# UBCMOCCA/mocca_envs

Hardware: AMD Instinct MI355X
Metric: env-steps/sec, Walker3DCustomEnv-v0 @ 4096 envs, 1/2/4/8 MI355X (higher is better)
Workload: dtype f32; 1 GPU; Walker3DCustomEnv-v0, 4096 envs/GPU, flat ground, U(-1,1) action tape, auto-reset; max_rows=48, max_contacts=12, envs_per_gpu=4096, parallelism=independent env shards x1, no collective, preroll_steps=6344

## Files before the change

### include/mocca.h

```cpp
#ifndef MOCCA_H
#define MOCCA_H

#include <stddef.h>
#include <stdint.h>

#include "mocca_model.h"

#ifdef __cplusplus
extern "C" {
#endif

#define MOCCA_ABI_VERSION 8

typedef struct mocca_ctx *mocca_handle;

enum {
  MOCCA_OK = 0,
  MOCCA_E_ARG = -1,
  MOCCA_E_HIP = -2,
  MOCCA_E_TOPOLOGY = -3,
  MOCCA_E_NODEVICE = -4,
};

enum {
  MOCCA_PARAM_AUTO_RESET = 0,
  MOCCA_PARAM_EVAL_MODE = 1,
  MOCCA_PARAM_CURRICULUM = 2,
  MOCCA_PARAM_RANDOM_POSE = 3,
  MOCCA_PARAM_HOST_RETARGET = 4,
  MOCCA_PARAM_SEED = 5,
  MOCCA_PARAM_ENV_OFFSET = 6,
  MOCCA_PARAM_RANDOM_REWARD = 8,
  MOCCA_PARAM_APPLIED_GAIN = 7,
  MOCCA_PARAM_ISSUE_PRIORITY = 9,
  MOCCA_PARAM_PERSIST_IMPULSES = 10,
  MOCCA_PARAM_KERNEL_VARIANT = 11,
  MOCCA_PARAM_ORDER_EVERY = 12,
  MOCCA_PARAM_PACE_TICKS = 13,
};

#define MOCCA_DEBUG_WORDS 20
enum {
  MOCCA_DBG_ROWS = 0,
  MOCCA_DBG_LIMIT_ROWS = 1,
  MOCCA_DBG_CONTACTS = 2,
  MOCCA_DBG_SLOTS_LO = 3,
  MOCCA_DBG_SLOTS_HI = 4,
  MOCCA_DBG_LIMITS_LO = 5,
  MOCCA_DBG_LIMITS_HI = 6,
  MOCCA_DBG_SELF = 7,
  MOCCA_DBG_CLAMP_LO = 8,
  MOCCA_DBG_CLAMP_HI = 9,
  MOCCA_DBG_CLAMPSIG_LO = 10,
  MOCCA_DBG_CLAMPSIG_HI = 11,
  MOCCA_DBG_CAP_CONTACTS = 12,
  MOCCA_DBG_CAP_ROWS = 13,
  MOCCA_DBG_SUBSTEPS = 14,
  MOCCA_DBG_ROWS_WANTED = 15,
  MOCCA_DBG_STEPSIG_LO = 16,
  MOCCA_DBG_STEPSIG_HI = 17,
  MOCCA_DBG_STEPSIG_N = 18,
  MOCCA_DBG_RESERVED = 19,
};

int mocca_abi_version(void);
size_t mocca_model_sizeof(void);

int mocca_create(const void *model_blob, size_t nbytes, int task_id, int n_envs, int device, mocca_handle *out);
int mocca_destroy(mocca_handle h);

int mocca_n_envs(mocca_handle h);
int mocca_obs_dim(mocca_handle h);
int mocca_act_dim(mocca_handle h);
int mocca_plan_dim(mocca_handle h);
int mocca_state_dim(mocca_handle h);

int mocca_reset(mocca_handle h, const uint8_t *mask_dev, uint64_t seed, float *obs_dev, void *stream);

int mocca_step(mocca_handle h, const float *act_dev, float *obs_dev, float *rew_dev, uint8_t *done_dev,
               int32_t *info_dev, void *stream);

int mocca_task_step(mocca_handle h, const float *act_dev, const int32_t *touch_dev, const int32_t *target_dev,
                    const int32_t *body_dev, float *obs_dev, float *rew_dev, uint8_t *done_dev, int32_t *info_dev,
                    void *stream);

int mocca_set_draw_tape(mocca_handle h, const float *tape_dev, int n_per_env);

int mocca_observe(mocca_handle h, float *obs_dev, void *stream);

int mocca_get_state(mocca_handle h, float *state_dev, void *stream);
int mocca_set_state(mocca_handle h, const float *state_dev, void *stream);
int mocca_get_task(mocca_handle h, uint32_t *task_dev, void *stream);
int mocca_set_task(mocca_handle h, const uint32_t *task_dev, void *stream);
int mocca_get_terrain(mocca_handle h, float *terrain_dev, void *stream);
int mocca_set_terrain(mocca_handle h, const float *terrain_dev, void *stream);

int mocca_set_param(mocca_handle h, int param_id, double value);
int mocca_set_param_v(mocca_handle h, int param_id, const float *values_dev, int broadcast, void *stream);
int mocca_set_seed(mocca_handle h, uint64_t seed);
int mocca_set_debug_buffer(mocca_handle h, int32_t *dbg_dev);
int mocca_set_terminal_obs_buffer(mocca_handle h, float *final_obs_dev);
typedef struct mocca_episode_rec {
  uint32_t serial;
  float ret;
  int32_t length;
  uint32_t flags;
} mocca_episode_rec;
int mocca_set_episode_stats(mocca_handle h, float *masks_dev, float *bad_masks_dev, float *totals_dev, void *records, int n_slots,
                            size_t slot_stride_bytes);
uint32_t mocca_episode_serial(mocca_handle h);

int mocca_is_diagnostic_build(void);

int mocca_set_trajectory(mocca_handle h, const float *table_host, int n_frames, double max_time, double control_step);

int mocca_set_heightfield(mocca_handle h, const float *heights_host, int rows, int cols, double scale);

#define MOCCA_HF_MAX_FIELDS 1024
#define MOCCA_HF_MAX_PEAKS 256
int mocca_set_heightfield_bank(mocca_handle h, const float *heights_host, int n_fields, int rows, int cols, double scale);
int mocca_generate_heightfields(mocca_handle h, int first, int count, uint64_t seed, int n_peaks, double gain, void *stream);
// ... 146 lines not shown
```

### mocca_envs_amd/csrc/mocca_api.hip

```cpp
#include <hip/hip_runtime.h>

#include <cmath>
#include <cstdio>
#include <cstring>
#include <functional>
#include <memory>
#include <new>
#include <string>
#include <utility>
#include <vector>

#include "mocca.h"
#include "mocca_kernels.h"
#include "mocca_optim.h"
#include "mocca_policy.h"
#include "mocca_ppo.h"
#include "mocca_render.h"
#include "mocca_rollout.h"
#include "mocca_scan.h"
#include "mocca_depth.h"
#include "mocca_terrain.h"
#include "mocca_randomise.h"

using namespace mocca;

extern "C" size_t mocca_r32_args_sizeof(void);
extern "C" int mocca_r32_max_rows(void);
extern "C" int mocca_r32_max_contacts(void);
extern "C" void mocca_r32_launch_step(int topo, int task_id, int n, hipStream_t s, const void* args);
extern "C" void mocca_r32_kernel_info(int topo, int task_id, hipFuncAttributes* fa, int* nb, hipError_t* e);
extern "C" size_t mocca_r64_args_sizeof(void);
extern "C" int mocca_r64_max_rows(void);
extern "C" int mocca_r64_max_contacts(void);
extern "C" void mocca_r64_launch_step(int topo, int task_id, int n, hipStream_t s, const void* args);
extern "C" void mocca_r64_kernel_info(int topo, int task_id, hipFuncAttributes* fa, int* nb, hipError_t* e);

__global__ void copy_param_kernel(float* dst, const float* src, bool broadcast, int n) {
  const int i = blockIdx.x * blockDim.x + threadIdx.x;
  if (i < n) dst[i] = src[broadcast ? 0 : i];
}
__global__ void set_task_word_kernel(uint32_t* task, int word, const float* vals, float scalar, int use_scalar, int n) {
  const int i = blockIdx.x * blockDim.x + threadIdx.x;
  if (i < n) task[(size_t)i * MOCCA_TASK_WORDS + word] = __float_as_uint(use_scalar ? scalar : vals[i]);
}

__global__ __launch_bounds__(1024) void order_by_rows_kernel(const uint32_t* task, int32_t* order, int n) {
  __shared__ int hist[64], start[64];
  const int t = threadIdx.x;
  if (t < 64) hist[t] = 0;
  __syncthreads();
  for (int e = t; e < n; e += 1024) {
    const uint32_t r = task[(size_t)e * MOCCA_TASK_WORDS + MOCCA_TW_LAST_ROWS];
    atomicAdd(&hist[63 - (r > 63u ? 63u : r)], 1);
  }
  __syncthreads();
  if (t == 0) {
    int acc = 0;
    for (int k = 0; k < 64; ++k) { start[k] = acc; acc += hist[k]; }
  }
  __syncthreads();
  for (int e = t; e < n; e += 1024) {
    const uint32_t r = task[(size_t)e * MOCCA_TASK_WORDS + MOCCA_TW_LAST_ROWS];
    order[atomicAdd(&start[63 - (r > 63u ? 63u : r)], 1)] = e;
  }
}

template <class T>
class DevBuf {
  T* p_ = nullptr;

 public:
  DevBuf() = default;
  DevBuf(DevBuf&& o) noexcept : p_(std::exchange(o.p_, nullptr)) {}
  DevBuf& operator=(DevBuf&& o) noexcept { swap(o); return *this; }
  ~DevBuf() { reset(); }
  void reset() {
    if (p_) (void)hipFree(p_);
    p_ = nullptr;
  }
  void swap(DevBuf& o) noexcept { std::swap(p_, o.p_); }
  hipError_t alloc(size_t count, bool zero) {
    reset();
    hipError_t e = hipMalloc(&p_, count * sizeof(T));
    if (e != hipSuccess) { p_ = nullptr; return e; }
    if (zero && (e = hipMemset(p_, 0, count * sizeof(T))) != hipSuccess) reset();
    return e;
  }
  T* get() const { return p_; }
  operator T*() const { return p_; }
};

struct mocca_ctx {
  MoccaModel model;
  int task_id = 0, n_envs = 0, device = 0, obs_dim = 0;
  DevBuf<MoccaModel> d_model;
  int topo = 0;
  DevBuf<float> d_dyn;
  DevBuf<uint32_t> d_task;
  DevBuf<float> d_terrain;
  int auto_reset = 0, eval_mode = 0, random_pose = 1, curriculum = 0, host_retarget = 0, env_offset = 0, random_reward = 0;
  float gain = 1.0f;
  bool compact = false;
  bool wide = false;
  int force_full = 0;
  bool delassus_valu = false;
  int persist_warm = 0;
  int pace = -18;
  DevBuf<unsigned long long> d_pace_acc;
  DevBuf<float> d_ep_ret;
  float *ep_masks = nullptr, *ep_bad = nullptr, *ep_totals = nullptr;
  char* ep_rec = nullptr;
  int ep_slots = 0;
  size_t ep_stride = 0;
  uint32_t ep_serial = 1;
  int order_every = 0;
  int order_age = 0;
  DevBuf<int32_t> d_order;
  bool gain_pending = false;
  float* final_obs = nullptr;
  DevBuf<float> d_pvec[3];
  bool pvec_on[3] = {false, false, false};
  const float* tape = nullptr;
  int tape_n = 0;
  int32_t* dbg = nullptr;
  int prio = MOCCA_PRIO_T1 + 64 * MOCCA_PRIO_T2 + 4096 * MOCCA_PRIO_T3;
  uint64_t seed = 0;
  DevBuf<float> d_traj;
  int traj_n = 0;
  double traj_tmax = 0.0, traj_cstep = 0.0;
  DevBuf<float> d_hf;
  int hf_rows = 0, hf_cols = 0, hf_n_fields = 0, hf_planes = 1;
  float hf_scale = 0.0f;
  DevBuf<float> d_hf_range;
  DevBuf<float> d_hf_part;
  DevBuf<int32_t> d_hf_field;
  int hf_redraw = 0;
  DevBuf<float> d_scenes;
  int scenes_cap = 0;
  DevBuf<float> d_scan_pts;
  int scan_n = 0;
  float scan_above = 0.0f, scan_drop = 0.0f;
  bool depth_on = false;
  mocca_depth::DepthArgs depth{};
  DevBuf<float> d_ctrl_image;
  DevBuf<int32_t> d_ctrl_layers;
  mocca_ctrl::ControllerArgs ctrl{};
  DevBuf<float> d_robot_state;
  DevBuf<float> d_base_act;
  DevBuf<float> d_base_val;
  DevBuf<float> d_ctrl_norm;
  struct PolicySlot {
    DevBuf<float> d_pol_image;
    DevBuf<int32_t> d_pol_layers;
    mocca_pol::PolicyArgs pol{};
    mocca_pol::RepackArgs pol_repack{};
    size_t pol_n_base = 0;
    bool pol_filled = false;
    int pol_tail_row = 0;
    std::vector<int32_t> pol_table;
    int pol_wt_off[mocca_ppo::PPO_MAX_TABLE] = {};
  } student, teacher;
  struct {
    mocca_ppo::PpoMode method = mocca_ppo::PPO_PLAIN;
    DevBuf<int32_t> perm;
    DevBuf<float> sign;
    double coef = 0.0;
  } pol_mirror;
  const float* critic_rows = nullptr;
  int critic_stride = 0;
  DevBuf<double> d_gae_part;
  size_t gae_part_cap = 0;
  DevBuf<double> d_obs_part;
  size_t obs_part_cap = 0;
  DevBuf<double> d_ppo;
  size_t ppo_cap = 0;
  DevBuf<double> d_optim;
  size_t optim_cap = 0;
  bool rand_on = false;
  mocca_rand::RandConfig rand_cfg{};
  DevBuf<float> d_rand_eff;
  DevBuf<float> d_rand_ring;
  DevBuf<float> d_noise_scale;
  std::string err;
};
static_assert(ROBOT_STATE_STRIDE == mocca_ctrl::CTRL_RS_STRIDE, "the step kernels and the controller kernel share the robot_state buffer");

static thread_local std::string g_err;

// ... 245 lines not shown
  int rc = check_topology(h->model, task_id, &h->topo, g_err);
  if (rc != MOCCA_OK) return rc;
  int ndev = 0;
  if (hipGetDeviceCount(&ndev) != hipSuccess || ndev <= 0 || device < 0 || device >= ndev) { g_err = "no such HIP device"; return MOCCA_E_NODEVICE; }
  h->task_id = task_id; h->n_envs = n_envs; h->device = device;
  h->compact = compact_ok(h->model, h->topo);
  h->wide = wide_needed(h->model);
  if (h->wide && mocca_r64_args_sizeof() != sizeof(StepArgs)) { g_err = "the 64-row kernel instance was built from another StepArgs"; return MOCCA_E_ARG; }
  if (h->compact) h->pace = 0;
  h->obs_dim = task_id == MOCCA_TASK_CASSIE
                   ? (h->model.cassie_mode == MOCCA_CASSIE_PLAIN ? 6 + 2 * h->model.n_ordered + 2 : 12 + 2 * h->model.n_ordered + 2)
                   : 6 + 2 * h->model.n_joints + h->model.n_feet + (task_id == MOCCA_TASK_WALKER3D_STEPPER ? 5 * (h->model.lookbehind + 2) : 2);
  if (task_id == MOCCA_TASK_CASSIE && (h->model.cassie_mode < MOCCA_CASSIE_PLAIN || h->model.cassie_mode > MOCCA_CASSIE_PHASE_MIRROR ||
                                       (h->model.cassie_mode != MOCCA_CASSIE_PLAIN && h->model.n_ordered != 14))) {
    g_err = "Cassie blob: unknown cassie_mode (the mocap / phase envs need the 14 ordered joints)"; return MOCCA_E_ARG;
  }
  if (task_id == MOCCA_TASK_WALKER3D_STEPPER &&
      (h->model.n_planks < 1 || h->model.n_planks > MOCCA_MAX_PLANKS || h->model.lookbehind < 1 || h->model.lookbehind > 2)) {
    g_err = "Stepper blob: n_planks must be 1..4 and lookbehind 1 or 2"; return MOCCA_E_ARG;
  }
  auto fail = [&](const char* what, hipError_t e) {
    g_err = std::string(what) + ": " + hipGetErrorString(e);
    return MOCCA_E_HIP;
  };
  hipError_t e;
  DeviceGuard guard(device);
  if ((e = guard.err) != hipSuccess) return fail("hipSetDevice", e);
  if ((e = h->d_model.alloc(1, false)) != hipSuccess) return fail("hipMalloc(model)", e);
  if ((e = hipMemcpy(h->d_model, &h->model, sizeof(MoccaModel), hipMemcpyHostToDevice)) != hipSuccess) return fail("hipMemcpy(model)", e);
  const size_t n = (size_t)n_envs;
  if ((e = h->d_dyn.alloc(n * DYN_STRIDE, false)) != hipSuccess) return fail("hipMalloc(state)", e);
  if ((e = h->d_task.alloc(n * MOCCA_TASK_WORDS, false)) != hipSuccess) return fail("hipMalloc(task)", e);
  if ((e = h->d_terrain.alloc(n * TERRAIN_STRIDE, true)) != hipSuccess) return fail("hipMalloc(terrain)", e);
  if ((e = h->d_pace_acc.alloc(1, true)) != hipSuccess) return fail("hipMalloc(pace samples)", e);
  {
    std::vector<uint32_t> tmp(n * MOCCA_TASK_WORDS);
    const float one = 1.0f;
    uint32_t one_bits; std::memcpy(&one_bits, &one, 4);
    for (size_t i = 0; i < n; ++i) {
      tmp[i * MOCCA_TASK_WORDS + MOCCA_TW_EPISODE] = (uint32_t)-1;
      tmp[i * MOCCA_TASK_WORDS + MOCCA_TW_APPLIED_GAIN] = one_bits;
    }
    if ((e = hipMemcpy(h->d_task, tmp.data(), tmp.size() * sizeof(uint32_t), hipMemcpyHostToDevice)) != hipSuccess) return fail("hipMemcpy(task)", e);
  }
  {
    std::vector<float> tmp(n * DYN_STRIDE);
    for (size_t i = 0; i < n; ++i) tmp[i * DYN_STRIDE + 6] = 1.0f;
    if ((e = hipMemcpy(h->d_dyn, tmp.data(), tmp.size() * sizeof(float), hipMemcpyHostToDevice)) != hipSuccess) return fail("hipMemcpy(state)", e);
  }
  *out = h.release();
  return MOCCA_OK;
} catch (const std::bad_alloc&) { return out_of_host_memory(nullptr, "mocca_create"); }

int mocca_destroy(mocca_handle h) {
  delete h;
  return MOCCA_OK;
}

int mocca_n_envs(mocca_handle h) { return h ? h->n_envs : MOCCA_E_ARG; }
int mocca_obs_dim(mocca_handle h) { return h ? h->obs_dim : MOCCA_E_ARG; }
int mocca_act_dim(mocca_handle h) {
  if (!h) return MOCCA_E_ARG;
  return h->task_id == MOCCA_TASK_CASSIE ? h->model.n_ctrl - 2 : h->model.n_joints;
}
int mocca_plan_dim(mocca_handle h) {
  if (!h) return MOCCA_E_ARG;
  if (h->task_id != MOCCA_TASK_WALKER3D_PLANNER) { h->err = "mocca_plan_dim: only the planner task takes plans"; return MOCCA_E_ARG; }
  return mocca_ctrl::CTRL_PLAN;
}
int mocca_state_dim(mocca_handle h) { return h ? MOCCA_STATE_DIM(h->model.n_joints, h->model.n_slots) : MOCCA_E_ARG; }

static StepArgs make_args(mocca_handle h) {
  StepArgs a{};
  a.model = h->d_model; a.dyn = h->d_dyn; a.task = h->d_task; a.terrain = h->d_terrain;
  a.n_envs = h->n_envs; a.obs_dim = h->obs_dim;
  a.auto_reset = h->auto_reset; a.eval_mode = h->eval_mode; a.random_pose = h->random_pose; a.curriculum = h->curriculum;
  a.host_retarget = h->host_retarget; a.env_offset = h->env_offset; a.random_reward = h->random_reward;
  a.seed_lo = (uint32_t)h->seed; a.seed_hi = (uint32_t)(h->seed >> 32);
  a.curriculum_v = h->pvec_on[0] ? h->d_pvec[0].get() : nullptr;
  a.eval_mode_v = h->pvec_on[1] ? h->d_pvec[1].get() : nullptr;
  a.gain_v = h->pvec_on[2] ? h->d_pvec[2].get() : nullptr;
  a.gain = h->gain;
  a.dbg = h->dbg;
  a.prio = h->prio | (h->delassus_valu ? PRIO_DELASSUS_VALU : 0);
  a.traj = h->d_traj; a.traj_n = h->traj_n; a.traj_tmax = h->traj_tmax; a.traj_cstep = h->traj_cstep;
  a.final_obs = h->final_obs;
  a.persist_warm = h->persist_warm;
  a.pace = h->pace;
  a.pace_acc = h->d_pace_acc;
  a.ep_ret = h->d_ep_ret; a.ep_masks = h->ep_masks; a.ep_bad = h->ep_bad; a.ep_totals = h->ep_totals;
  a.hf = h->d_hf; a.hf_rows = h->hf_rows; a.hf_cols = h->hf_cols; a.hf_scale = h->hf_scale;
  if (h->hf_n_fields > 1) {
    a.hf_field = h->d_hf_field; a.hf_stride = h->hf_planes * h->hf_rows * h->hf_cols; a.hf_n_fields = h->hf_n_fields; a.hf_redraw = h->hf_redraw;
  }
  a.robot_state = h->d_ctrl_image ? h->d_robot_state.get() : nullptr;
  return a;
}
static int flush_pending(mocca_handle h, hipStream_t s) {
  if (!h->gain_pending) return MOCCA_OK;
  launch_per_env(set_task_word_kernel, h, s, h->d_task, MOCCA_TW_APPLIED_GAIN, nullptr, h->gain, 1, h->n_envs);
  HIP_TRY(h, hipGetLastError());
  h->gain_pending = false;
  return MOCCA_OK;
}
static int need_heightfield(mocca_handle h, const char* who, const char* when) {
  if (h->task_id != MOCCA_TASK_WALKER3D_PLANNER || h->d_hf) return MOCCA_OK;
  h->err = std::string(who) + "the planner task needs mocca_set_heightfield " + when;
  return MOCCA_E_ARG;
}
static mocca_rdr::HeightFieldBank heightfield_record(mocca_handle h) {
  if (h->task_id != MOCCA_TASK_WALKER3D_PLANNER) return mocca_rdr::HeightFieldBank{nullptr, 0, 0, 0.0f, nullptr, nullptr, 0};
  return mocca_rdr::HeightFieldBank{h->d_hf, h->hf_rows, h->hf_cols, h->hf_scale, h->d_hf_range, h->hf_n_fields > 1 ? h->d_hf_field.get() : nullptr,
                                    (size_t)h->hf_planes * h->hf_rows * h->hf_cols};
}
static int need_attachments(mocca_handle h) {
  if (h->task_id == MOCCA_TASK_CASSIE && h->model.cassie_mode != MOCCA_CASSIE_PLAIN && !h->d_traj) {
    h->err = "this Cassie blob (cassie_mode != 0) needs mocca_set_trajectory before reset / step / observe";
    return MOCCA_E_ARG;
  }
  return need_heightfield(h, "", "before reset / step / observe");
}

int mocca_reset(mocca_handle h, const uint8_t* mask_dev, uint64_t seed, float* obs_dev, void* stream) {
  if (!h || !obs_dev) return MOCCA_E_ARG;
  if (need_attachments(h) != MOCCA_OK) return MOCCA_E_ARG;
  h->seed = seed;
  DeviceGuard guard(h->device);
  StepArgs a = make_args(h);
  a.mask = mask_dev; a.obs = obs_dev;
  hipStream_t s = (hipStream_t)stream;
  if (int rc = flush_pending(h, s)) return rc;
  if (h->tape) {
    a.tape = h->tape; a.tape_n = h->tape_n;
    launch_taped_reset(h->topo, h->task_id, h->n_envs, s, a);
  } else {
    dispatch<LaunchReset>(h->topo, h->task_id, h->n_envs, s, a);
  }
  HIP_TRY(h, hipGetLastError());
  return MOCCA_OK;
}

static mocca_rand::RandKeys rand_keys(mocca_handle h) {
  return mocca_rand::RandKeys{h->d_task, MOCCA_TASK_WORDS, MOCCA_TW_T, MOCCA_TW_EPISODE, h->env_offset, h->n_envs, (uint32_t)h->seed,
                              (uint32_t)(h->seed >> 32)};
}

static int launch_step(mocca_handle h, const float* act_dev, const float* base_value, float* obs_dev, float* rew_dev, uint8_t* done_dev,
                       int32_t* info_dev, hipStream_t s) {
  StepArgs a = make_args(h);
  a.act = act_dev; a.obs = obs_dev; a.rew = rew_dev; a.done = done_dev; a.info = info_dev;
  a.base_value = base_value;
  if (int rc = flush_pending(h, s)) return rc;
  if (h->rand_on) {
    mocca_rand::PerturbArgs p{rand_keys(h), h->rand_cfg, act_dev, h->d_rand_eff, h->d_rand_ring, h->d_dyn, DYN_STRIDE, mocca_act_dim(h)};
    mocca_rand::launch_perturb(s, p);
    HIP_TRY(h, hipGetLastError());
    a.act = h->d_rand_eff;
  }
  if (h->d_ep_ret && h->ep_rec) {
    a.ep_rec = h->ep_rec + (size_t)(h->ep_serial % (uint32_t)h->ep_slots) * h->ep_stride;
    a.ep_serial = h->ep_serial;
    if (++h->ep_serial == 0u) h->ep_serial = 1u;
  }
  if (h->order_every > 0 && h->d_order) {
    if (h->order_age >= h->order_every) {
      hipLaunchKernelGGL(order_by_rows_kernel, dim3(1), dim3(1024), 0, s, (const uint32_t*)h->d_task, h->d_order, h->n_envs);
      HIP_TRY(h, hipGetLastError());
// ... 470 lines not shown
}

int mocca_get_state(mocca_handle h, float* state_dev, void* stream) {
  if (!h || !state_dev) return MOCCA_E_ARG;
  DeviceGuard guard(h->device);
  const size_t w = (size_t)mocca_state_dim(h) * sizeof(float);
  HIP_TRY(h, hipMemcpy2DAsync(state_dev, w, h->d_dyn, DYN_STRIDE * sizeof(float), w, h->n_envs, hipMemcpyDeviceToDevice,
                              (hipStream_t)stream));
  return MOCCA_OK;
}
int mocca_set_state(mocca_handle h, const float* state_dev, void* stream) {
  if (!h || !state_dev) return MOCCA_E_ARG;
  DeviceGuard guard(h->device);
  const size_t w = (size_t)mocca_state_dim(h) * sizeof(float);
  HIP_TRY(h, hipMemcpy2DAsync(h->d_dyn, DYN_STRIDE * sizeof(float), state_dev, w, w, h->n_envs, hipMemcpyDeviceToDevice,
                              (hipStream_t)stream));
  return MOCCA_OK;
}
int mocca_get_task(mocca_handle h, uint32_t* task_dev, void* stream) {
  if (!h || !task_dev) return MOCCA_E_ARG;
  DeviceGuard guard(h->device);
  if (int rc = flush_pending(h, (hipStream_t)stream)) return rc;
  HIP_TRY(h, hipMemcpyAsync(task_dev, h->d_task, (size_t)h->n_envs * MOCCA_TASK_WORDS * 4, hipMemcpyDeviceToDevice, (hipStream_t)stream));
  return MOCCA_OK;
}
int mocca_set_task(mocca_handle h, const uint32_t* task_dev, void* stream) {
  if (!h || !task_dev) return MOCCA_E_ARG;
  DeviceGuard guard(h->device);
  h->gain_pending = false;
  HIP_TRY(h, hipMemcpyAsync(h->d_task, task_dev, (size_t)h->n_envs * MOCCA_TASK_WORDS * 4, hipMemcpyDeviceToDevice, (hipStream_t)stream));
  return MOCCA_OK;
}
int mocca_get_terrain(mocca_handle h, float* terrain_dev, void* stream) {
  if (!h || !terrain_dev) return MOCCA_E_ARG;
  DeviceGuard guard(h->device);
  HIP_TRY(h, hipMemcpyAsync(terrain_dev, h->d_terrain, (size_t)h->n_envs * TERRAIN_STRIDE * 4, hipMemcpyDeviceToDevice, (hipStream_t)stream));
  return MOCCA_OK;
}
int mocca_set_terrain(mocca_handle h, const float* terrain_dev, void* stream) {
  if (!h || !terrain_dev) return MOCCA_E_ARG;
  DeviceGuard guard(h->device);
  HIP_TRY(h, hipMemcpyAsync(h->d_terrain, terrain_dev, (size_t)h->n_envs * TERRAIN_STRIDE * 4, hipMemcpyDeviceToDevice, (hipStream_t)stream));
  return MOCCA_OK;
}

int mocca_set_param(mocca_handle h, int param_id, double value) {
  if (!h) return MOCCA_E_ARG;
  switch (param_id) {
    case MOCCA_PARAM_AUTO_RESET: h->auto_reset = value != 0; break;
    case MOCCA_PARAM_EVAL_MODE: h->eval_mode = value != 0; h->pvec_on[1] = false; break;
    case MOCCA_PARAM_CURRICULUM: h->curriculum = (int)value < 0 ? 0 : ((int)value > 9 ? 9 : (int)value); h->pvec_on[0] = false; break;
    case MOCCA_PARAM_APPLIED_GAIN:
      h->gain = (float)value; h->pvec_on[2] = false; h->gain_pending = true;
      break;
    case MOCCA_PARAM_RANDOM_POSE: h->random_pose = value != 0; break;
    case MOCCA_PARAM_HOST_RETARGET: h->host_retarget = value != 0; break;
    case MOCCA_PARAM_SEED: h->seed = (uint64_t)value; break;
    case MOCCA_PARAM_ENV_OFFSET: h->env_offset = (int)value; break;
    case MOCCA_PARAM_ISSUE_PRIORITY:
      if (value < 0 || value >= 262144) { h->err = "MOCCA_PARAM_ISSUE_PRIORITY is t1 + 64 t2 + 4096 t3 with each threshold in 0..63"; return MOCCA_E_ARG; }
      h->prio = (int)value;
      break;
    case MOCCA_PARAM_RANDOM_REWARD:
      if (value != 0 && value != 1 && value != 2) { h->err = "MOCCA_PARAM_RANDOM_REWARD is 0, 1 or 2"; return MOCCA_E_ARG; }
      h->random_reward = (int)value; break;
    case MOCCA_PARAM_PERSIST_IMPULSES: h->persist_warm = value != 0; break;
    case MOCCA_PARAM_PACE_TICKS:
      if (value < -64 || value > 1e9) { h->err = "MOCCA_PARAM_PACE_TICKS is a tick count > 0, 0 (off) or -k (self-calibrating, k / 16 of the mean wave time, k <= 64)"; return MOCCA_E_ARG; }
      h->pace = (int)value; break;
    case MOCCA_PARAM_ORDER_EVERY:
      if (value < 0 || value > 1e6) { h->err = "MOCCA_PARAM_ORDER_EVERY is a step count >= 0"; return MOCCA_E_ARG; }
      h->order_every = (int)value; h->order_age = h->order_every;
      if (h->order_every > 0 && !h->d_order) {
        DeviceGuard guard(h->device);
        HIP_TRY(h, h->d_order.alloc((size_t)h->n_envs, false));
      }
      break;
    case MOCCA_PARAM_KERNEL_VARIANT: {
      if (value != (double)(int)value || value < 0 || value > 7 || ((int)value & 3) == 3) { h->err = "MOCCA_PARAM_KERNEL_VARIANT is 0 (automatic), 1 (force the 48-row instance) or 2 (force the 64-row instance), plus 4 to build the Delassus matrix on the VALU"; return MOCCA_E_ARG; }
      const int inst = (int)value & 3;
      if (inst == 1 && h->wide) { h->err = "MOCCA_PARAM_KERNEL_VARIANT = 1: this blob needs the 64-row instance (caps beyond 48 rows / 12 contacts, or sweep_alternate)"; return MOCCA_E_ARG; }
      h->force_full = inst; h->delassus_valu = ((int)value & 4) != 0; break;
    }
    default: h->err = "unknown parameter id"; return MOCCA_E_ARG;
  }
  return MOCCA_OK;
}

int mocca_set_param_v(mocca_handle h, int param_id, const float* values_dev, int broadcast, void* stream) {
  if (!h || !values_dev) return MOCCA_E_ARG;
  const int slot = param_id == MOCCA_PARAM_CURRICULUM ? 0 : param_id == MOCCA_PARAM_EVAL_MODE ? 1 : param_id == MOCCA_PARAM_APPLIED_GAIN ? 2 : -1;
  if (slot < 0) { h->err = "this parameter has no per-env form"; return MOCCA_E_ARG; }
  DeviceGuard guard(h->device);
  if (!h->d_pvec[slot]) HIP_TRY(h, h->d_pvec[slot].alloc((size_t)h->n_envs, false));
  hipStream_t s = (hipStream_t)stream;
  launch_per_env(copy_param_kernel, h, s, h->d_pvec[slot], values_dev, broadcast != 0, h->n_envs);
  HIP_TRY(h, hipGetLastError());
  if (slot == 2) {
    h->gain_pending = false;
    launch_per_env(set_task_word_kernel, h, s, h->d_task, MOCCA_TW_APPLIED_GAIN, h->d_pvec[slot], 0.0f, 0, h->n_envs);
    HIP_TRY(h, hipGetLastError());
  }
  h->pvec_on[slot] = true;
  return MOCCA_OK;
}

static mocca_rdr::SceneArgs scene_args(mocca_handle h) {
  mocca_rdr::SceneArgs a{};
  a.model = h->d_model; a.dyn = h->d_dyn; a.task = h->d_task; a.terrain = h->d_terrain;
  a.dyn_stride = DYN_STRIDE; a.terrain_stride = TERRAIN_STRIDE; a.task_id = h->task_id;
  return a;
}

int mocca_get_link_frames(mocca_handle h, float* frames_dev, void* stream) {
  if (!h || !frames_dev) return MOCCA_E_ARG;
  DeviceGuard guard(h->device);
  mocca_rdr::launch_link_frames((hipStream_t)stream, scene_args(h), h->n_envs, frames_dev);
  HIP_TRY(h, hipGetLastError());
  return MOCCA_OK;
}

int mocca_render(mocca_handle h, const int32_t* env_ids_dev, int n_views, const float* cameras_dev, int width, int height, uint8_t* rgb_dev,
                 float* depth_dev, int32_t* id_dev, void* stream) try {
  if (!h) return MOCCA_E_ARG;
  if (!env_ids_dev || !cameras_dev) { h->err = "mocca_render: env_ids_dev and cameras_dev must not be NULL"; return MOCCA_E_ARG; }
  if (n_views < 1 || n_views > 65535) { h->err = "mocca_render: n_views must be 1 .. 65535"; return MOCCA_E_ARG; }
  if (width < 1 || height < 1 || width > MOCCA_RENDER_MAX_SIZE || height > MOCCA_RENDER_MAX_SIZE) {
    h->err = "mocca_render: width and height must be 1 .. " + std::to_string(MOCCA_RENDER_MAX_SIZE); return MOCCA_E_ARG;
  }
  if (need_heightfield(h, "mocca_render: ", "first") != MOCCA_OK) return MOCCA_E_ARG;
  DeviceGuard guard(h->device);
  hipStream_t s = (hipStream_t)stream;
  std::vector<int32_t> ids((size_t)n_views);
  HIP_TRY(h, hipMemcpyAsync(ids.data(), env_ids_dev, ids.size() * sizeof(int32_t), hipMemcpyDeviceToHost, s));
  HIP_TRY(h, hipStreamSynchronize(s));
  for (int v = 0; v < n_views; ++v)
    if (ids[v] < 0 || ids[v] >= h->n_envs) {
      h->err = "mocca_render: env index " + std::to_string(ids[v]) + " (view " + std::to_string(v) + ") is outside 0 .. " + std::to_string(h->n_envs - 1);
      return MOCCA_E_ARG;
    }
  if (n_views > h->scenes_cap) {
    DevBuf<float> scenes;
    if (int rc = commit_ready(h, "mocca_render", scenes.alloc((size_t)n_views * mocca_rdr::SCENE_WORDS, false))) return rc;
    h->d_scenes.swap(scenes);
    h->scenes_cap = n_views;
  }
  if (int rc = flush_pending(h, s)) return rc;
  mocca_rdr::launch_scene(s, scene_args(h), env_ids_dev, h->n_envs, n_views, h->d_scenes);
  HIP_TRY(h, hipGetLastError());
  mocca_rdr::launch_raycast(s, h->d_scenes, cameras_dev, n_views, width, height, h->task_id, h->model.plank_shape, h->model.plank_half,
                            heightfield_record(h), env_ids_dev, rgb_dev, depth_dev, id_dev);
  HIP_TRY(h, hipGetLastError());
  return MOCCA_OK;
} catch (const std::bad_alloc&) { return out_of_host_memory(h, "mocca_render"); }

int mocca_set_height_scan(mocca_handle h, const float* points_host, int n_points, double z_above, double max_drop) {
  if (!h) return MOCCA_E_ARG;
  DeviceGuard guard(h->device);
  if (!points_host) {
    if (int rc = commit_ready(h, "mocca_set_height_scan")) return rc;
    h->d_scan_pts.reset(); h->scan_n = 0;
    return MOCCA_OK;
  }
  auto bad = [&](const std::string& what) { h->err = "mocca_set_height_scan: " + what; return MOCCA_E_ARG; };
  if (n_points < 1 || n_points > MOCCA_SCAN_MAX_POINTS) return bad("n_points must be 1 .. " + std::to_string(MOCCA_SCAN_MAX_POINTS));
  if (!std::isfinite(z_above) || !std::isfinite(max_drop) || z_above < 0.0 || !(max_drop > 0.0)) return bad("needs a finite z_above >= 0 and max_drop > 0");
// ... 737 lines not shown
```

### mocca_envs_amd/csrc/mocca_device.h

```cpp
#pragma once

#include <hip/hip_runtime.h>
#include <stdint.h>

#include "mocca_model.h"
#include "mocca_philox.h"
#include "topo_walker3d.h"
#include "topo_cassie.h"
#include "topo_walker2d.h"
#include "topo_crab2d.h"
#include "topo_laikago.h"

#define DI __device__ __forceinline__

#ifndef MOCCA_NS
#define MOCCA_NS mocca
#endif
#ifndef MOCCA_MAXR
#define MOCCA_MAXR 48
#endif
#ifndef MOCCA_COMPACT
#define MOCCA_COMPACT 0
#endif

// ... 118 lines not shown
    if (T::cchild(b, k) >= 0) return true;
  return false;
}

enum : int { C_BA = 0, C_BB = 1, C_SLOT = 2, C_P = 3, C_N = 6, C_DEPTH = 9, C_MU = 10, C_ERP = 11, C_CFM = 12, C_MA = 13, C_MB = 14 };

struct StepArgs {
  const MoccaModel* model;
  float* dyn;
  uint32_t* task;
  float* terrain;
  const float* act;
  float* obs;
  float* rew;
  uint8_t* done;
  int32_t* info;
  const uint8_t* mask;
  int n_envs;
  int obs_dim;
  int auto_reset;
  int eval_mode;
  int random_pose;
  int curriculum;
  int host_retarget;
  int env_offset;
  uint32_t seed_lo, seed_hi;
  const float* curriculum_v;
  const float* eval_mode_v;
  int random_reward;
  const float* gain_v;
  float gain;
  const int32_t* inj_touch;
  const int32_t* inj_target;
  const int32_t* inj_body;
  const float* tape;
  int tape_n;
  int32_t* dbg;
  const float* traj;
  int traj_n;
  double traj_tmax, traj_cstep;
  int prio;
  const float* hf;
  int hf_rows, hf_cols;
  float hf_scale;
  float* final_obs;
  int persist_warm;
  const int32_t* order;
  int pace;
  unsigned long long* pace_acc;
  float* ep_ret;
  float* ep_masks;
  float* ep_bad;
  void* ep_rec;
  float* ep_totals;
  uint32_t ep_serial;
  float* robot_state;
  const float* base_value;
  int32_t* hf_field;
  int hf_stride, hf_n_fields, hf_redraw;
};
constexpr int ROBOT_STATE_STRIDE = 64;

DI void read_kernargs(StepArgs& la) {
  auto p = __builtin_amdgcn_kernarg_segment_ptr();
  asm volatile("" : "+s"(p));
  __builtin_memcpy(&la, p, sizeof(StepArgs));
}
template <bool LATE>
DI void late_args(StepArgs& la) {
  if constexpr (LATE) read_kernargs(la);
}
template <class T>
#ifdef MOCCA_NO_TRIM_8
constexpr bool OUTWARD_ROUNDS = false;
#else
constexpr bool OUTWARD_ROUNDS = T::OUTWARD_DPP && !COMPACT;
#endif
template <class T>
#ifdef MOCCA_NO_TRIM_9
constexpr bool WALK_LEVELS = false;
#else
constexpr bool WALK_LEVELS = OUTWARD_ROUNDS<T>;
#endif
template <class T>
constexpr int walk_base_lane() {
  for (int l = 63; l >= 0; --l)
    if (T::out_body(l) < 0) return l;
  return -1;
}
template <class T, int TASK, bool INJECT>
#ifdef MOCCA_NO_TRIM_7
constexpr bool LATE_ARGS = false;
#else
constexpr bool LATE_ARGS = INJECT || MAXR > 48 || !__is_base_of(TopoWalker3D, T) || (!COMPACT && TASK == MOCCA_TASK_WALKER3D_CUSTOM);
#endif

DI void wsync() {
  __builtin_amdgcn_fence(__ATOMIC_RELEASE, "wavefront");
  __builtin_amdgcn_wave_barrier();
  __builtin_amdgcn_fence(__ATOMIC_ACQUIRE, "wavefront");
}
DI float dot3(const float* a, const float* b) { return a[0] * b[0] + a[1] * b[1] + a[2] * b[2]; }
DI void cross3(const float* a, const float* b, float* o) {
  float x = a[1] * b[2] - a[2] * b[1], y = a[2] * b[0] - a[0] * b[2], z = a[0] * b[1] - a[1] * b[0];
  o[0] = x; o[1] = y; o[2] = z;
}
DI float dot6(const float* a, const float* b) {
  return a[0] * b[0] + a[1] * b[1] + a[2] * b[2] + a[3] * b[3] + a[4] * b[4] + a[5] * b[5];
}
DI void matvec3(const float* R, const float* x, float* o) {
  float a = R[0] * x[0] + R[1] * x[1] + R[2] * x[2];
  float b = R[3] * x[0] + R[4] * x[1] + R[5] * x[2];
  float c = R[6] * x[0] + R[7] * x[1] + R[8] * x[2];
  o[0] = a; o[1] = b; o[2] = c;
}
DI void matmul3(const float* A, const float* B, float* C) {
  float T[9];
#pragma unroll
  for (int i = 0; i < 3; ++i)
#pragma unroll
    for (int j = 0; j < 3; ++j) T[3 * i + j] = A[3 * i] * B[j] + A[3 * i + 1] * B[3 + j] + A[3 * i + 2] * B[6 + j];
#pragma unroll
  for (int i = 0; i < 9; ++i) C[i] = T[i];
}
DI void quat_to_mat(const float* q, float* R) {
  float x = q[0], y = q[1], z = q[2], w = q[3];
  R[0] = 1 - 2 * (y * y + z * z); R[1] = 2 * (x * y - z * w); R[2] = 2 * (x * z + y * w);
  R[3] = 2 * (x * y + z * w); R[4] = 1 - 2 * (x * x + z * z); R[5] = 2 * (y * z - x * w);
  R[6] = 2 * (x * z - y * w); R[7] = 2 * (y * z + x * w); R[8] = 1 - 2 * (x * x + y * y);
}
DI void crm(const float* v, const float* m, float* o) {
  float a[3], b[3], c[3];
  cross3(v, m, a); cross3(v, m + 3, b); cross3(v + 3, m, c);
  o[0] = a[0]; o[1] = a[1]; o[2] = a[2];
  o[3] = b[0] + c[0]; o[4] = b[1] + c[1]; o[5] = b[2] + c[2];
}
DI void crf(const float* v, const float* f, float* o) {
  float a[3], b[3], c[3];
  cross3(v, f, a); cross3(v + 3, f + 3, b); cross3(v, f + 3, c);
  o[0] = a[0] + b[0]; o[1] = a[1] + b[1]; o[2] = a[2] + b[2];
  o[3] = c[0]; o[4] = c[1]; o[5] = c[2];
}
DI constexpr int sym(int i, int j) { return i <= j ? i * 6 - i * (i - 1) / 2 + (j - i) : j * 6 - j * (j - 1) / 2 + (i - j); }
DI void symmv6(const float* A, const float* x, float* o) {
#pragma unroll
  for (int i = 0; i < 6; ++i) {
    float s = 0;
#pragma unroll
    for (int j = 0; j < 6; ++j) s += A[sym(i, j)] * x[j];
    o[i] = s;
  }
}
DI void spatial_inertia_mv(const float* A, const float* x, float* o) {
  constexpr unsigned long long Z = (1ull << 3) | (1ull << 10) | (1ull << 17) | (1ull << 18) | (1ull << 22) | (1ull << 23) |
                                   (1ull << 25) | (1ull << 27) | (1ull << 29) | (1ull << 32) | (1ull << 33) | (1ull << 34);
#pragma unroll
  for (int i = 0; i < 6; ++i) {
    float s = 0;
#pragma unroll
    for (int j = 0; j < 6; ++j)
      if (!((Z >> (6 * i + j)) & 1ull)) s += A[sym(i, j)] * x[j];
    o[i] = s;
  }
}
DI float rcp(float x) { return __builtin_amdgcn_rcpf(x); }
DI float rsq(float x) { return __builtin_amdgcn_rsqf(x); }
DI void pin6(float* v) { asm volatile("" : "+v"(v[0]), "+v"(v[1]), "+v"(v[2]), "+v"(v[3]), "+v"(v[4]), "+v"(v[5])); }
DI void pin1(float& v) { asm volatile("" : "+v"(v)); }
template <int CTRL>
DI float dpp_mov(float v) {
  return __builtin_bit_cast(float, __builtin_amdgcn_update_dpp(0, __builtin_bit_cast(int, v), CTRL, 0xF, 0xF, true));
}
DI float group8_sum(float t) {
  t += dpp_mov<0xB1>(t);
  t += dpp_mov<0x4E>(t);
  t += dpp_mov<0x141>(t);
  return t;
}
DI void group8_sum2(float& a, float& b) {
  asm("s_nop 1\n\t"
      "v_add_f32_dpp %0, %0, %0 quad_perm:[1,0,3,2] row_mask:0xf bank_mask:0xf\n\t"
      "v_add_f32_dpp %1, %1, %1 quad_perm:[1,0,3,2] row_mask:0xf bank_mask:0xf\n\t"
      "s_nop 0\n\t"
      "v_add_f32_dpp %0, %0, %0 quad_perm:[2,3,0,1] row_mask:0xf bank_mask:0xf\n\t"
      "v_add_f32_dpp %1, %1, %1 quad_perm:[2,3,0,1] row_mask:0xf bank_mask:0xf\n\t"
      "s_nop 0\n\t"
      "v_add_f32_dpp %0, %0, %0 row_half_mirror row_mask:0xf bank_mask:0xf\n\t"
      "v_add_f32_dpp %1, %1, %1 row_half_mirror row_mask:0xf bank_mask:0xf"
      : "+v"(a), "+v"(b));
}
DI int uni(int v) { return __builtin_amdgcn_readfirstlane(v); }
DI float unif(float v) { return __builtin_bit_cast(float, __builtin_amdgcn_readfirstlane(__builtin_bit_cast(int, v))); }
DI float readlane(float v, int l) { return __builtin_bit_cast(float, __builtin_amdgcn_readlane(__builtin_bit_cast(int, v), l)); }
DI int readlane_i(int v, int l) { return __builtin_amdgcn_readlane(v, l); }
template <int LANE>
DI float writelane_c(float v, float old) {
  asm("v_writelane_b32 %0, %1, %2" : "+v"(old) : "s"(v), "n"(LANE));
  return old;
}
template <int LANE>
DI float commit_lane(float v, float old) {
  float r;
  unsigned long long m;
  if constexpr (LANE < 31)
    asm("s_mov_b64 %1, %4\n\tv_cndmask_b32 %0, %2, %3, %1" : "=v"(r), "=&s"(m) : "v"(old), "v"(v), "n"(1u << LANE));
  else
    asm("s_mov_b64 %1, 0\n\ts_bitset1_b64 %1, %4\n\tv_cndmask_b32 %0, %2, %3, %1" : "=v"(r), "=&s"(m) : "v"(old), "v"(v), "n"(LANE));
  return r;
}
DI int lane_rank(unsigned long long mask) {
  return __builtin_amdgcn_mbcnt_hi((unsigned)(mask >> 32), __builtin_amdgcn_mbcnt_lo((unsigned)mask, 0));
}
template <int CTRL>
DI unsigned dpp_or(unsigned v) { return v | (unsigned)__builtin_amdgcn_update_dpp(0, (int)v, CTRL, 0xF, 0xF, true); }
DI unsigned wave_or(unsigned v) {
  v = dpp_or<0xB1>(v);
  v = dpp_or<0x4E>(v);
  v = dpp_or<0x141>(v);
  v = dpp_or<0x140>(v);
  return (unsigned)(readlane_i((int)v, 0) | readlane_i((int)v, 16) | readlane_i((int)v, 32) | readlane_i((int)v, 48));
}
DI float wave_sum(float v) {
  v += dpp_mov<0xB1>(v);
  v += dpp_mov<0x4E>(v);
  v += dpp_mov<0x141>(v);
  v += dpp_mov<0x140>(v);
  return (readlane(v, 0) + readlane(v, 16)) + (readlane(v, 32) + readlane(v, 48));
}

DI float wave_max(float v) {
  v = fmaxf(v, dpp_mov<0xB1>(v));
  v = fmaxf(v, dpp_mov<0x4E>(v));
  v = fmaxf(v, dpp_mov<0x141>(v));
  v = fmaxf(v, dpp_mov<0x140>(v));
  return fmaxf(fmaxf(readlane(v, 0), readlane(v, 16)), fmaxf(readlane(v, 32), readlane(v, 48)));
}

DI float rng_uniform(uint32_t slo, uint32_t shi, uint32_t env, uint32_t episode, uint32_t d) {
  uint32_t o[4];
  philox4x32(d >> 2, episode, env, 0u, slo, shi, o);
  uint32_t w = (d & 3) == 0 ? o[0] : (d & 3) == 1 ? o[1] : (d & 3) == 2 ? o[2] : o[3];
  return (float)(w >> 8) * (1.0f / 16777216.0f);
}

template <bool INJECT>
DI float draw_u(const StepArgs& a, int env, int episode, int d) {
  if constexpr (INJECT) {
    if (a.tape) return d < a.tape_n ? a.tape[(size_t)(env - a.env_offset) * a.tape_n + d] : 0.5f;
  }
  return rng_uniform(a.seed_lo, a.seed_hi, (uint32_t)env, (uint32_t)episode, (uint32_t)d);
}
// ... 1000 lines not shown
    const unsigned long long hm = __ballot(hit);
    if (TASK == MOCCA_TASK_WALKER3D_PLANNER && hm != 0ull) {
      int tor = 0;
      if (hit) { const int ids2 = __float_as_int((*(CF4P)(M->pair_tab[cand[base + lane]])).x); tor = M->g_torso[ids2 & 31] | M->g_torso[(ids2 >> 5) & 31]; }
      if (__ballot(hit && tor) != 0ull) fl.body_touch = 1;
    }
    if (TASK == MOCCA_TASK_WALKER3D_STEPPER) {
      const int f0 = M->foot_body[0], f1 = M->foot_body[1];
      if (__ballot(hit && (ba == f0 || bb == f0)) != 0ull) fl.touch0 = 1;
      if (__ballot(hit && (ba == f1 || bb == f1)) != 0ull) fl.touch1 = 1;
      if constexpr (T::NFEET > 2) {
        const int f2 = M->foot_body[2], f3 = M->foot_body[3];
        if (__ballot(hit && (ba == f2 || bb == f2)) != 0ull) fl.touch2 = 1;
        if (__ballot(hit && (ba == f3 || bb == f3)) != 0ull) fl.touch3 = 1;
      }
    }
    const int idx = nc + lane_rank(hm);
    if (hit && idx < maxc) {
      float* ct = L + L_CT + 16 * idx;
      ct[C_BA] = __int_as_float(ba); ct[C_BB] = __int_as_float(bb); ct[C_SLOT] = __int_as_float(-1);
#pragma unroll
      for (int i = 0; i < 3; ++i) { ct[C_P + i] = PP[i]; ct[C_N + i] = nn[i]; }
      ct[C_DEPTH] = -g2; ct[C_MU] = mu2; ct[C_ERP] = M->erp; ct[C_CFM] = 0.0f;
      ct[C_MA] = __uint_as_float(M->anc_mask[ba]); ct[C_MB] = __uint_as_float(M->anc_mask[bb]);
    }
    nc += __popcll(hm);
    n_self += __popcll(hm);
    if (nc > maxc) nc = maxc;
  }
  STAMP(14);
  if (dbg && lane == 0) {
    dbg[3] = (int32_t)(unsigned)am; dbg[4] = (int32_t)(unsigned)(am >> 32); dbg[7] = n_self;
  }
  *nc_out = nc;
  *nc_wanted = n_terrain + n_self;
  return fl;
}

template <class T, int TT>
DI void delassus_dots(const float* L, const float* X, int oc, int onr, int tmax, float* v) {
  if constexpr (TT <= MAXR / 2) {
    if (TT > tmax) return;
    const unsigned o = (unsigned)(oc + 28 * TT);
    const unsigned ow = o - (unsigned)onr;
    const float* Jr = L + L_J + (int)(o < ow ? o : ow);
    float s;
    if constexpr (T::NCLOS > 0) {
      float s0 = 0, s1 = 0;
#pragma unroll
      for (int d = 0; d + 1 < T::ND; d += 2) { s0 += Jr[d] * X[d]; s1 += Jr[d + 1] * X[d + 1]; }
      if constexpr (T::ND & 1) s0 += Jr[T::ND - 1] * X[T::ND - 1];
      s = s0 + s1;
    } else {
      s = 0;
#pragma unroll
      for (int d = 0; d < T::ND; ++d) s += Jr[d] * X[d];
    }
    v[TT] = s;
    pin1(v[TT]);
    delassus_dots<T, TT + 1>(L, X, oc, onr, tmax, v);
  }
}
template <int TT>
DI void delassus_store(float* L, int c, int nr, int tmax, const float* v) {
  if constexpr (TT <= MAXR / 2) {
    if (TT > tmax) return;
    const unsigned r0 = (unsigned)(c + TT), rw = r0 - (unsigned)nr;
    const int rho = (int)(r0 < rw ? r0 : rw);
    if (TT == 0) {
      L[L_A + (MAXR + 1) * c] = 0.0f;
    } else {
      L[L_A + __mul24(MAXR, rho) + c] = v[TT];
      L[L_A + __mul24(MAXR, c) + rho] = v[TT];
    }
    delassus_store<TT + 1>(L, c, nr, tmax, v);
  }
}

constexpr int DELASSUS_MFMA_ROWS = COMPACT ? 16 : 32;
#ifndef MOCCA_DELASSUS_MFMA_MIN
#define MOCCA_DELASSUS_MFMA_MIN 8
#endif
constexpr int PRIO_DELASSUS_VALU = 1 << 18;
enum : int { L_DX = L_V };
static_assert(L_DX + 28 * DELASSUS_MFMA_ROWS <= L_J && MAXR >= DELASSUS_MFMA_ROWS, "the X rows of the matrix-pipe Delassus build end before the J rows");
template <int R, int C>
DI void delassus_tile_store(float* L, const f4_t& acc, int nr, int li, int lk) {
  const int c = 16 * C + li;
#pragma unroll
  for (int j = 0; j < 4; ++j) {
    const int r = 16 * R + 4 * lk + j;
    int e = r - c;
    if (e < 0) e += nr;
    const bool in = r < nr && c < nr;
    if (in && 2 * e <= nr) L[L_A + __mul24(MAXR, c) + r] = acc[j];
    if (in && 2 * e < nr) L[L_A + __mul24(MAXR, r) + c] = acc[j];
  }
}
template <class T>
DI float delassus_mfma(float* L, const float* X, int cc, bool has_row, int nr, int lane) {
  if (has_row) {
    int xo = 28 * cc;
    asm volatile("" : "+v"(xo));
    float* xr = L + L_DX + xo;
#pragma unroll
    for (int d = 0; d < 28; ++d) xr[d] = d < T::ND ? X[d < T::ND ? d : 0] : 0.0f;
  }
  wsync();
  asm volatile("" : "+v"(lane));
  const int li = lane & 15, lk = lane >> 4;
  const float* Jl = L + L_J + 28 * li + lk;
  const float* Xl = L + L_DX + 28 * li + lk;
  f4_t d00 = {0.0f, 0.0f, 0.0f, 0.0f};
  bool four = false;
  if constexpr (DELASSUS_MFMA_ROWS > 16) four = nr > 16;
  if (!four) {
#pragma unroll
    for (int kk = 0; kk < 7; ++kk) d00 = __builtin_amdgcn_mfma_f32_16x16x4f32(Jl[4 * kk], Xl[4 * kk], d00, 0, 0, 0);
    wsync();
    delassus_tile_store<0, 0>(L, d00, nr, li, lk);
  } else {
    f4_t d01 = d00, d10 = d00, d11 = d00;
#pragma unroll
    for (int kk = 0; kk < 7; ++kk) {
      const float j0 = Jl[4 * kk], j1 = Jl[28 * 16 + 4 * kk], x0 = Xl[4 * kk], x1 = Xl[28 * 16 + 4 * kk];
      d00 = __builtin_amdgcn_mfma_f32_16x16x4f32(j0, x0, d00, 0, 0, 0);
      d01 = __builtin_amdgcn_mfma_f32_16x16x4f32(j0, x1, d01, 0, 0, 0);
      d10 = __builtin_amdgcn_mfma_f32_16x16x4f32(j1, x0, d10, 0, 0, 0);
      d11 = __builtin_amdgcn_mfma_f32_16x16x4f32(j1, x1, d11, 0, 0, 0);
    }
    wsync();
    delassus_tile_store<0, 0>(L, d00, nr, li, lk);
    delassus_tile_store<0, 1>(L, d01, nr, li, lk);
    delassus_tile_store<1, 0>(L, d10, nr, li, lk);
    delassus_tile_store<1, 1>(L, d11, nr, li, lk);
  }
  wsync();
  float diag = 1.0f;
  if (has_row) {
    diag = L[L_A + (MAXR + 1) * cc];
    L[L_A + (MAXR + 1) * cc] = 0.0f;
  }
  return diag;
}

template <int RR>
DI void pgs_visit(float as, float& y, float& lam, float lo0) {
  const float nl_ = __builtin_amdgcn_fmed3f(y, lo0, 1e30f);
  const float dl = readlane(nl_ - lam, RR);
  lam = commit_lane<RR>(nl_, lam);
  y = fmaf(-as, dl, y);
}
template <int RR>
DI void pgs_visit_friction(float as, float& y, float& lam, float lm) {
  const float nl_ = __builtin_amdgcn_fmed3f(y, -lm, lm);
  const float dl = readlane(nl_ - lam, RR);
  lam = commit_lane<RR>(nl_, lam);
  y = fmaf(-as, dl, y);
}
template <int A>
DI float commit_pair(float v, float old) {
  float r;
  unsigned long long m;
  asm("s_mov_b64 %1, 0\n\ts_bitset1_b64 %1, %4\n\ts_bitset1_b64 %1, %5\n\tv_cndmask_b32 %0, %2, %3, %1"
      : "=v"(r), "=&s"(m) : "v"(old), "v"(v), "n"(A), "n"(A + 1));
  return r;
// ... 65 lines not shown
      if constexpr (RR + 4 >= PGS_REG_ROWS) { pin1(n0); pin1(n1); pin1(n2); pin1(n3); }
      pgs_fixed_rows<PGS_REG_ROWS, RR + 4>(Acol, ar, n0, n1, n2, n3, r_fr, y, lam, invdiag, lo0);
      return;
    }
  }
  pgs_fixed_tail<PGS_REG_ROWS, RR, 3>(ar, a0, a1, a2, r_fr, y, lam, invdiag, lo0);
}

DI void pgs_reverse_rows(const float* Acol, int nnc, int lane, float& y, float& lam, float invdiag, float lo0) {
#pragma unroll 1
  for (int j = nnc - 1; j >= 0; --j) {
    const float as = Acol[MAXR * j] * invdiag;
    const float nl_ = __builtin_amdgcn_fmed3f(y, lo0, 1e30f);
    const float dl = readlane(nl_ - lam, j);
    lam = lane == j ? nl_ : lam;
    y = fmaf(-as, dl, y);
  }
}
template <int PGS_REG_ROWS, int RR>
DI void pgs_fixed_rows_from(const float* Acol, const float* ar, int start, int r_fr, float& y, float& lam, float invdiag, float lo0) {
  if constexpr (RR < MAXR) {
    if (RR >= r_fr) return;
    if (RR >= start) pgs_visit<RR>(RR < PGS_REG_ROWS ? ar[RR < PGS_REG_ROWS ? RR : 0] : Acol[MAXR * RR] * invdiag, y, lam, lo0);
    pgs_fixed_rows_from<PGS_REG_ROWS, RR + 1>(Acol, ar, start, r_fr, y, lam, invdiag, lo0);
  }
}

DI void set_issue_priority(int nr, int prio) {
  if (nr > ((prio >> 12) & 63)) __builtin_amdgcn_s_setprio(3);
  else if (nr > ((prio >> 6) & 63)) __builtin_amdgcn_s_setprio(2);
  else if (nr > (prio & 63)) __builtin_amdgcn_s_setprio(1);
  else __builtin_amdgcn_s_setprio(0);
}
#ifndef MOCCA_PACE_ROWUNIT
#define MOCCA_PACE_ROWUNIT 2
#endif
#ifndef MOCCA_PACE_SHIFT
#define MOCCA_PACE_SHIFT 4
#endif
constexpr int PACE_TICK_SHIFT = 6;
enum : int { L_T0 = L_BASE + 13, L_PACE = L_BASE + 14, L_KEEPWARM = L_BASE + 15  };
constexpr unsigned PACE_CNT_BITS = 24, PACE_WINDOW = 128;
DI void pace_start(const StepArgs& a, float* L, int lane, int pace) {
  if (lane == 0) {
    int p16 = pace >> PACE_TICK_SHIFT;
    if (pace < 0) {
      const unsigned long long v = __hip_atomic_load(a.pace_acc, __ATOMIC_RELAXED, __HIP_MEMORY_SCOPE_AGENT);
      const unsigned cnt = (unsigned)v & ((1u << PACE_CNT_BITS) - 1u);
      p16 = cnt > 0u ? (int)((float)(v >> PACE_CNT_BITS) / (float)cnt * (float)(-pace) * 0.0625f) : 0;
    }
    L[L_PACE] = __int_as_float(p16);
    if (pace != 0) L[L_T0] = __uint_as_float((unsigned)__builtin_amdgcn_s_memtime());
  }
}
DI void pace_finish(const StepArgs& a, const float* L, int lane, int pace) {
  if (pace < 0 && lane == 0 && (blockIdx.x % 61u) == 0u) {
    const unsigned el = ((unsigned)__builtin_amdgcn_s_memtime() - __float_as_uint(L[L_T0])) >> PACE_TICK_SHIFT;
    const unsigned long long old = atomicAdd(a.pace_acc, ((unsigned long long)el << PACE_CNT_BITS) | 1ull);
    if (((unsigned)old & ((1u << PACE_CNT_BITS) - 1u)) + 1u == PACE_WINDOW) {
      const unsigned long long sum = (old >> PACE_CNT_BITS) + el;
      atomicAdd(a.pace_acc, 0ull - (((sum >> 1) << PACE_CNT_BITS) | (unsigned long long)(PACE_WINDOW / 2)));
    }
  }
}
DI bool pace_on(const float* L) { return uni(__float_as_int(L[L_PACE])) > 0; }
DI void pace_checkpoint(const float* L, int done, int total) {
  const unsigned p16 = (unsigned)uni(__float_as_int(L[L_PACE]));
  if (p16 == 0u) return;
  const unsigned el = (unsigned)__builtin_amdgcn_s_memtime() - (unsigned)uni(__float_as_int(L[L_T0]));
  const unsigned lhs = (el >> PACE_TICK_SHIFT) * (unsigned)total, r = p16 * (unsigned)done;
  if (lhs > r + (r >> MOCCA_PACE_SHIFT)) __builtin_amdgcn_s_setprio(3);
  else if (lhs > r) __builtin_amdgcn_s_setprio(2);
  else if (lhs > r - (r >> MOCCA_PACE_SHIFT)) __builtin_amdgcn_s_setprio(1);
  else __builtin_amdgcn_s_setprio(0);
}
DI void dbg_fold_step(int32_t* dbg, int lane) {
  if (dbg && lane == 0) {
    unsigned long long h = ((unsigned long long)(unsigned)dbg[17] << 32) | (unsigned)dbg[16];
#pragma unroll 1
    for (int w = 0; w < 12; ++w) h = (h ^ (unsigned long long)(unsigned)dbg[w]) * 0x9E3779B97F4A7C15ull;
    dbg[16] = (int32_t)(unsigned)h; dbg[17] = (int32_t)(unsigned)(h >> 32); dbg[18] += 1;
  }
}
template <class T, bool MATRIX_PIPE>
DI void solve_constraints(ModelP M, float* L, int lane, int nc_found, int nc_wanted, unsigned long long ppk, int32_t* dbg, const float* Afac, int prio, int& rows_out) {
  const int wave_flags = uni(__float_as_int(L[L_KEEPWARM]));
  const bool keep_warm = (wave_flags & 1) != 0;
  STAMP_BEGIN;
  const float dt = unif(M->dt), idt = rcp(dt);
  const int maxr = uni(M->max_rows);
  int nl;
  {
    bool act = false;
    float gap = 0.0f;
    if (lane < 2 * T::NJ) {
      const int b = 1 + (lane >> 1), side = lane & 1;
      const float q = L[L_Q + b];
      gap = side == 0 ? q - M->jlo[b] : M->jhi[b] - q;
      const float vel = (side == 0 ? 1.0f : -1.0f) * L[L_NU + 5 + b];
      act = M->limit_at_violation ? !(gap > 0.0f) : gap + dt * vel < M->limit_slack;
    }
    const unsigned long long lm = __ballot(act);
    const int rk = lane_rank(lm);
    if (act && rk < maxr) {
      reinterpret_cast<int*>(L)[L_ROWD + rk] = lane;
#ifndef MOCCA_NO_TRIM_2
      L[L_LGAP + rk] = gap;
#endif
    }
    nl = uni(__popcll(lm));
    if (dbg && lane == 0) {
      dbg[5] = (int32_t)(unsigned)lm; dbg[6] = (int32_t)(unsigned)(lm >> 32);
      const int nfix = 3 * T::NCLOS + ((T::NCLOS > 0 && M->planar) ? 3 : 0), mc = M->max_contacts;
      const int wanted = nl + nfix + 3 * nc_wanted;
      dbg[12] += nc_wanted > mc ? 1 : 0;
      dbg[13] += nl + nfix + 3 * (nc_wanted < mc ? nc_wanted : mc) > maxr ? 1 : 0;
      dbg[14] += 1;
      if (wanted > dbg[15]) dbg[15] = wanted;
    }
    if (nl > maxr) nl = maxr;
  }
  constexpr int NCL = 3 * T::NCLOS;
  const int NFIX = NCL + ((T::NCLOS > 0 && uni(M->planar)) ? 3 : 0);
  int nc = uni(nc_found);
  if (nc > (maxr - nl - NFIX) / 3) nc = (maxr - nl - NFIX) / 3;
  if (nc < 0) nc = 0;
  const int nr = nl + NFIX + 3 * nc;
  if (dbg && lane == 0) { dbg[0] = nr; dbg[1] = nl; dbg[2] = nc; }
  if (!pace_on(L)) set_issue_priority(nr, prio);
  rows_out = nr;
  wsync();
  STAMP(16);
  if (nr == 0) {
    if (dbg && lane == 0) { dbg[8] = 0; dbg[9] = 0; dbg[10] = 0; dbg[11] = 0; }
    if (keep_warm && lane < T::NSLOT) L[L_WARM + lane] = 0.0f;
    wsync();
    return;
  }
  const int r = lane;
  const int r_fr = nl + NFIX + nc;
  const int row_gap = MAXR - nr;
  const bool is_fric = r >= MAXR - 2 * nc && r < MAXR;
  const bool has_row = r < r_fr || is_fric;
  const int ci = is_fric ? (MAXR - 1 - r) >> 1 : r - nl - NFIX;
  int kind = -1, ba = 0, bb = -1, jl = -1, slot = -1;
  float F[6] = {0, 0, 0, 0, 0, 0}, sgn = 0, bias = 0, cfm = 0, lam = 0, mu = 0;
  float F2[6] = {0, 0, 0, 0, 0, 0};
  if (r < nl) {
    const int c = reinterpret_cast<int*>(L)[L_ROWD + r];
    const int b = 1 + (c >> 1), side = c & 1;
#ifndef MOCCA_NO_TRIM_2
    const float gap = L[L_LGAP + r];
#else
    const float q = L[L_Q + b];
    const float gap = side == 0 ? q - M->jlo[b] : M->jhi[b] - q;
#endif
    kind = 0; jl = b; ba = b; sgn = side == 0 ? 1.0f : -1.0f;
    bias = gap < 0 ? M->erp_noncontact * (-gap) * idt : -gap * idt;
  } else if (T::NCLOS > 0 && r < nl + NCL) {
    const int c = (r - nl) / 3, ax = (r - nl) % 3;
    ba = M->cl_body_a[c]; bb = M->cl_body_b[c];
    kind = 3;
    float Pa[3], Pb[3], Ra[9], Rb[9], la[3], lb[3];
#pragma unroll
    for (int x = 0; x < 9; ++x) { Ra[x] = L[L_RT + 12 * ba + 4 * (x / 3) + x % 3]; Rb[x] = L[L_RT + 12 * bb + 4 * (x / 3) + x % 3]; }
#pragma unroll
    for (int x = 0; x < 3; ++x) { la[x] = M->cl_point_a[c][x]; lb[x] = M->cl_point_b[c][x]; }
// ... 61 lines not shown
  const int dense = has_row ? (r < r_fr ? r : r - row_gap) : MAXR;
  float* Jrow = L + L_J + 28 * dense;
  float pa[6] = {0, 0, 0, 0, 0, 0}, pb[6] = {0, 0, 0, 0, 0, 0};
#ifdef MOCCA_NO_TWO_PATHS
  const bool two_paths = false;
#else
  const bool two_paths = T::NCLOS > 0 || __ballot(kind >= 1 && bb >= 0) != 0ull;
#endif
  STAMP(18);
  const unsigned long long pka = ((unsigned long long)(unsigned)__shfl((int)(unsigned)(ppk >> 32), ba, 64) << 32) |
                                 (unsigned long long)(unsigned)__shfl((int)(unsigned)ppk, ba, 64);
  {
    float4* jz = reinterpret_cast<float4*>(Jrow);
#pragma unroll
    for (int i = 1; i < 7; ++i) jz[i] = make_float4(0.0f, 0.0f, 0.0f, 0.0f);
  }
  float pu[T::MAXD], pub[T::MAXD];
#pragma unroll
  for (int k = T::MAXD - 1; k >= 0; --k) {
    const int j = (int)((pka >> (5 * k)) & 31ull);
    const bool valid = j != 0;
    const int jj = j;
    float S[6], U[6];
#pragma unroll
    for (int i = 0; i < 6; ++i) { S[i] = L[L_SV + SVS * jj + i]; U[i] = L[L_SV + SVS * jj + SV_V + i]; }
    float jb = dot6(S, F);
    if (jj == jl) jb = sgn;
    jb = valid ? jb : 0.0f;
    const float uu = valid ? (k == T::MAXD - 1 ? jb : jb - dot6(S, pa)) : 0.0f;
#pragma unroll
    for (int i = 0; i < 6; ++i) pa[i] += U[i] * uu;
    if (valid) Jrow[5 + jj] = jb;
    w += jb * L[L_NU + 5 + jj];
    pu[k] = uu * L[L_SV + SVS * jj + SV_INVD];
    pin6(pa); pin1(pu[k]); pin1(w);
  }
  if (two_paths) {
    const int bq = bb >= 0 ? bb : 0;
    const unsigned long long pkb = ((unsigned long long)(unsigned)__shfl((int)(unsigned)(ppk >> 32), bq, 64) << 32) |
                                   (unsigned long long)(unsigned)__shfl((int)(unsigned)ppk, bq, 64);
#pragma unroll
    for (int k = T::MAXD - 1; k >= 0; --k) {
      const int j = (int)((pkb >> (5 * k)) & 31ull);
      const bool valid = j != 0;
      const int jj = j;
      float S[6], U[6];
#pragma unroll
      for (int i = 0; i < 6; ++i) { S[i] = L[L_SV + SVS * jj + i]; U[i] = L[L_SV + SVS * jj + SV_V + i]; }
      const float jb = valid ? -dot6(S, F2) : 0.0f;
      const float uu = valid ? (k == T::MAXD - 1 ? jb : jb - dot6(S, pb)) : 0.0f;
#pragma unroll
      for (int i = 0; i < 6; ++i) pb[i] += U[i] * uu;
      if (valid) Jrow[5 + jj] += jb;
      w += jb * L[L_NU + 5 + jj];
      pub[k] = uu * L[L_SV + SVS * jj + SV_INVD];
      pin6(pb); pin1(pub[k]); pin1(w);
    }
  }
#ifdef MOCCA_NO_TRIM_5
  else {
#pragma unroll
    for (int k = 0; k < T::MAXD; ++k) pub[k] = 0.0f;
  }
#endif
  STAMP(19);
  int l2off = 0;
  asm volatile("" : "+v"(l2off));
  l2off &= ~3;
  const float* L2 = L + l2off;
  float a0[6];
  {
    float rhs[6];
#pragma unroll
    for (int i = 0; i < 6; ++i) {
      const float jb = F[i] * sa - F2[i] * sb;
      Jrow[i] = jb;
      w += jb * L[L_NU + i];
      rhs[i] = jb - (pa[i] + pb[i]);
    }
    chol6_solve(Afac, rhs, a0);
#pragma unroll
    for (int i = 0; i < 6; ++i) X[i] = a0[i];
  }
  {
    float acc[T::NB][6];
#pragma unroll
    for (int i = 0; i < 6; ++i) acc[0][i] = a0[i];
#pragma unroll
    for (int b = 1; b < T::NB; ++b) {
      const int p = T::parent(b);
#ifdef MOCCA_NO_TRIM_4
      constexpr bool inner = true;
#else
      const bool inner = has_child<T>(b);
#endif
      float U[6];
#pragma unroll
      for (int i = 0; i < 6; ++i) U[i] = L2[L_SV + SVS * b + SV_V + i];
      const int dpos = T::depth(b) - 1;
      float ub = __uint_as_float(__float_as_uint(pu[dpos]) & (unsigned)__builtin_amdgcn_sbfe((int)ma, b, 1));
      if (two_paths) ub += __uint_as_float(__float_as_uint(pub[dpos]) & (unsigned)__builtin_amdgcn_sbfe((int)mb, b, 1));
      const float qdd = ub - dot6(U, acc[p]);
      X[5 + b] = qdd;
      if (inner) {
        float S[6];
#pragma unroll
        for (int i = 0; i < 6; ++i) { S[i] = L2[L_SV + SVS * b + i]; acc[b][i] = acc[p][i] + S[i] * qdd; }
        pin6(acc[b]);
      }
      pin1(X[5 + b]);
    }
  }
  STAMP(6);
  wsync();
  const int lc = has_row ? dense : MAXR - 1;
  float diag;
  bool on_mfma = false;
  if constexpr (T::NCLOS == 0 && MATRIX_PIPE) on_mfma = nr >= MOCCA_DELASSUS_MFMA_MIN && nr <= DELASSUS_MFMA_ROWS && !(wave_flags & 2);
  if (on_mfma) {
    diag = delassus_mfma<T>(L, X, has_row ? dense : 0, has_row, nr, lane);
  } else {
    float av[MAXR / 2 + 1];
    const int cc = has_row ? dense : 0, tmax = nr >> 1;
    delassus_dots<T, 0>(L, X, 28 * cc, 28 * nr, tmax, av);
    diag = has_row ? av[0] : 1.0f;
    wsync();
    if (has_row) delassus_store<0>(L, cc, nr, tmax, av);
  }
  const float invdiag = diag + cfm > 1e-12f ? rcp(diag + cfm) : 0.0f;
  wsync();
  STAMP(7);
  if (__ballot(lam != 0.0f) != 0ull) {
    int rr = nl + NFIX;
    const int rend = nl + NFIX + nc;
#pragma unroll 1
    for (; rr + 2 <= rend; rr += 2) {
      const float g0 = L[L_A + MAXR * rr + lc], g1 = L[L_A + MAXR * rr + MAXR + lc];
      w += g0 * readlane(lam, rr); w += g1 * readlane(lam, rr + 1);
    }
    if (rr < rend) w += L[L_A + MAXR * rr + lc] * readlane(lam, rr);
  }
  STAMP(20);
  const int iters = uni(M->n_iters);
  const bool cone = uni(M->friction_cone) != 0;
  const float lo0 = kind == 3 ? -1e30f : 0.0f;
  const float* Acol = L + L_A + lc;
  const float* Acol_fr = Acol - MAXR * row_gap;
  const int nrow_lane = is_fric ? nl + NFIX + ci : 0;
  float y = (bias - w) * invdiag;
  constexpr int PGS_REG_ROWS = PgsWin<T>::ROWS, PGS_REG_CONTACTS = PgsWin<T>::CONTACTS;
  static_assert(PGS_REG_ROWS % 4 == 0 && PGS_REG_ROWS <= MAXR && PGS_REG_CONTACTS <= MAXC, "register window of the solver");
  float ar[PGS_REG_ROWS], af[2 * PGS_REG_CONTACTS];
#pragma unroll
  for (int k = 0; k < PGS_REG_ROWS; ++k) ar[k] = Acol[MAXR * k] * invdiag;
#pragma unroll
  for (int k = 0; k < PGS_REG_CONTACTS; ++k) {
    af[2 * k] = 0.0f; af[2 * k + 1] = 0.0f;
    if (k < nc) { af[2 * k] = Acol_fr[MAXR * fric_lane(k, 0)] * invdiag; af[2 * k + 1] = Acol_fr[MAXR * fric_lane(k, 1)] * invdiag; }
  }
  unsigned long long clamp_sig = 0ull, clamp_last = 0ull;
  const int nnc = nl + NFIX;
  const bool alt = ALT_SWEEPS && uni(M->sweep_alternate) != 0 && nnc > 1;
#pragma unroll 1
  for (int it = 0; it < iters; ++it) {
    int rf = r_fr, ncc = nc;
    asm volatile("" : "+s"(rf), "+s"(ncc));
    bool fwd = true;
    if constexpr (ALT_SWEEPS) {
      if (alt && !(it & 1)) {
        int nn = nnc;
        asm volatile("" : "+s"(nn));
        pgs_reverse_rows(Acol, nn, lane, y, lam, invdiag, lo0);
        pgs_fixed_rows_from<PGS_REG_ROWS, 0>(Acol, ar, nn, rf, y, lam, invdiag, lo0);
        fwd = false;
      }
    }
    if (fwd) pgs_fixed_rows<PGS_REG_ROWS, 0>(Acol, ar, 0.0f, 0.0f, 0.0f, 0.0f, rf, y, lam, invdiag, lo0);
    float lm = 0.0f;
    if (ncc > 0) {
      float f0 = 0.0f, f1 = 0.0f, g0 = 0.0f, g1 = 0.0f;
      if (PGS_REG_CONTACTS < 1) { f0 = Acol_fr[MAXR * fric_lane(0, 0)]; f1 = Acol_fr[MAXR * fric_lane(0, 1)]; }
      if (PGS_REG_CONTACTS < 2 && ncc > 1) { g0 = Acol_fr[MAXR * fric_lane(1, 0)]; g1 = Acol_fr[MAXR * fric_lane(1, 1)]; }
      const float ln_ = __shfl(lam, nrow_lane, 64);
      lm = mu * ln_;
      const unsigned long long fpos = __ballot(ln_ > 0.0f);
      if (cone) pgs_friction_rows<PGS_REG_ROWS, PGS_REG_CONTACTS, 0, true>(Acol_fr, af, f0, f1, g0, g1, ncc, y, lam, invdiag, lm, fpos);
      else pgs_friction_rows<PGS_REG_ROWS, PGS_REG_CONTACTS, 0, false>(Acol_fr, af, f0, f1, g0, g1, ncc, y, lam, invdiag, lm, fpos);
    }
    if (dbg) {
      const float lpart = __shfl_xor(lam, 1, 64);
// ... 92 lines not shown
}

#ifdef MOCCA_NO_TRIM_6
template <class T, bool AXES_ = true>
DI void stage_joints(ModelP M, float* L, int lane) {
  constexpr bool AXES = true;
#else
template <class T, bool AXES = true>
DI void stage_joints(ModelP M, float* L, int lane) {
#endif
  if (lane < T::NB) {
    const int j = lane;
    float s, cq;
    fast_sincos(L[L_Q + j], &s, &cq);
    const float t = 1.0f - cq;
    float ax[3], jr[9], Rq[9], Tl[9];
#pragma unroll
    for (int i = 0; i < 3; ++i) ax[i] = M->jaxis[j][i];
#pragma unroll
    for (int i = 0; i < 9; ++i) jr[i] = M->jrot[j][i];
    Rq[0] = cq + t * ax[0] * ax[0];          Rq[1] = t * ax[0] * ax[1] - s * ax[2];   Rq[2] = t * ax[0] * ax[2] + s * ax[1];
    Rq[3] = t * ax[0] * ax[1] + s * ax[2];   Rq[4] = cq + t * ax[1] * ax[1];          Rq[5] = t * ax[1] * ax[2] - s * ax[0];
    Rq[6] = t * ax[0] * ax[2] - s * ax[1];   Rq[7] = t * ax[1] * ax[2] + s * ax[0];   Rq[8] = cq + t * ax[2] * ax[2];
    matmul3(jr, Rq, Tl);
    float4* rec = reinterpret_cast<float4*>(L + L_SV + SVS * j);
    rec[0] = make_float4(Tl[0], Tl[1], Tl[2], Tl[3]);
    rec[1] = make_float4(Tl[4], Tl[5], Tl[6], Tl[7]);
    rec[2] = make_float4(Tl[8], M->jpos[j][0], M->jpos[j][1], M->jpos[j][2]);
    if constexpr (AXES) rec[3] = make_float4(ax[0], ax[1], ax[2], L[L_QD + j]);
  }
  wsync();
}

template <class T, int TASK>
DI ContactFlags substep(ModelP M, float* L, int lane, const float* ter, int next_step_index,
                        unsigned long long ppk, int32_t* dbg, int prio, int& rows_out,
                        const HeightFieldArgs hfa = HeightFieldArgs{nullptr, 0, 0, 0.0f}, int sidx = 0, int nsub = 1, int* cover_out = nullptr) {
  const int per0 = 64 + MOCCA_PACE_ROWUNIT * rows_out, done0 = sidx * per0, total = nsub * per0;
  STAMP(30);
  stage_joints<T>(M, L, lane);
  STAMP(29);
  int nc = 0, nc_wanted = 0;
  float Afac[21] = {0, 0, 0, 0, 0, 0, 0, 0, 0, 0, 0, 0, 0, 0, 0, 0, 0, 0, 0, 0, 0};
  ContactFlags fl = {0, 0, 0, 0, 0, 0, 0, 0, 0};
  if constexpr (COMPACT) {
    static_assert(!COMPACT || T::NCLOS == 0, "closure rows read the body frames after the ABA: not in the compact layout");
    int wl = lane;
    asm volatile("" : "+v"(wl));
    walk_phase1<T>(L, wl, ppk);
    wsync();
    STAMP(0);
    geom_points<T>(M, L, lane);
    wsync();
    STAMP(15);
#ifndef MOCCA_SKIP_COLLIDE
    fl = collide<T, TASK>(M, L, lane, ter, next_step_index, &nc, dbg, &nc_wanted, hfa, cover_out);
#endif
    wsync();
    const int wb = wl < T::NB ? wl : 0;
    WalkConsts wk;
    walk_consts<true>(M, wb, wk);
    walk_phase2<T, true>(M, L, wl, wb, ppk, wk);
    wsync();
  } else {
    walk_kinematics<T, true>(M, L, lane, ppk);
    wsync();
    STAMP(0);
    geom_points<T>(M, L, lane);
    wsync();
    STAMP(15);
#ifndef MOCCA_SKIP_COLLIDE
    fl = collide<T, TASK>(M, L, lane, ter, next_step_index, &nc, dbg, &nc_wanted, hfa, cover_out);
#endif
  }
  STAMP(1);
  pace_checkpoint(L, done0 + 20, total);
  constexpr bool PLANNER48 = !COMPACT && MAXR == 48 && TASK == MOCCA_TASK_WALKER3D_PLANNER;
#ifndef MOCCA_SKIP_ABA
  aba_passes<T, !PLANNER48>(M, L, lane, ppk, Afac);
#endif
  STAMP(2);
  pace_checkpoint(L, done0 + 36, total);
#ifndef MOCCA_SKIP_SOLVE
  solve_constraints<T, !PLANNER48>(M, L, lane, nc, nc_wanted, ppk, dbg, Afac, prio, rows_out);
#endif
  if (dbg) { __builtin_amdgcn_s_waitcnt(0); dbg_fold_step(dbg, lane); }
  STAMP(3);
#ifdef MOCCA_DUMMY_VALU
  {
    float x = (float)lane;
#ifdef MOCCA_DUMMY_ILP
    float y = x + 1.0f, z = x + 2.0f, u = x + 3.0f;
#pragma unroll 1
    for (int i = 0; i < MOCCA_DUMMY_VALU; ++i) { x = fmaf(x, 1.0001f, 0.5f); y = fmaf(y, 0.9999f, -0.5f); z = fmaf(z, 1.0001f, 0.5f); u = fmaf(u, 0.9999f, -0.5f); }
    asm volatile("" :: "v"(y), "v"(z), "v"(u));
#else
#pragma unroll 1
    for (int i = 0; i < MOCCA_DUMMY_VALU; ++i) { x = fmaf(x, 1.0001f, 0.5f); x = fmaf(x, 0.9999f, -0.5f); x = fmaf(x, 1.0001f, 0.5f); x = fmaf(x, 0.9999f, -0.5f); }
#endif
    asm volatile("" :: "v"(x));
  }
#endif
  integrate<T>(M, L, lane);
  STAMP(4);
  pace_checkpoint(L, (sidx + 1) * (64 + MOCCA_PACE_ROWUNIT * rows_out), nsub * (64 + MOCCA_PACE_ROWUNIT * rows_out));
  return fl;
}

DI void quat_to_rpy(const float* q, float* rpy) {
  const float x = q[0], y = q[1], z = q[2], w = q[3];
  const float sarg = -2 * (x * z - w * y);
  if (sarg <= -0.99999f) { rpy[1] = -1.5707963267948966f; rpy[0] = 0; rpy[2] = 2 * atan2f(x, -y); }
  else if (sarg >= 0.99999f) { rpy[1] = 1.5707963267948966f; rpy[0] = 0; rpy[2] = 2 * atan2f(-x, y); }
  else {
    rpy[0] = atan2f(2 * (y * z + w * x), w * w - x * x - y * y + z * z);
    rpy[1] = asinf(sarg);
    rpy[2] = atan2f(2 * (x * y + w * z), w * w + x * x - y * y - z * z);
  }
}

DI void quat_to_rp_heading(const float* q, float* rp, float* cy, float* sy) {
  const float x = q[0], y = q[1], z = q[2], w = q[3];
  const float sarg = -2 * (x * z - w * y);
  if (sarg <= -0.99999f) { rp[1] = -1.5707963267948966f; rp[0] = 0; const float yaw = 2 * atan2f(x, -y); *cy = cosf(yaw); *sy = sinf(yaw); }
  else if (sarg >= 0.99999f) { rp[1] = 1.5707963267948966f; rp[0] = 0; const float yaw = 2 * atan2f(-x, y); *cy = cosf(yaw); *sy = sinf(yaw); }
  else {
    rp[0] = atan2f(2 * (y * z + w * x), w * w - x * x - y * y + z * z);
    rp[1] = asinf(sarg);
    const float A = 2 * (x * y + w * z), B = w * w + x * x - y * y - z * z, n = rsq(A * A + B * B);
    *cy = B * n; *sy = A * n;
  }
}

template <class T> constexpr int ROBOT_OBS = 6 + 2 * T::NJ + T::NFEET;
struct RobotObs { float rpy[3];  float cy, sy; int jal; float spd; float height; bool finite; };

template <class T>
DI RobotObs robot_obs(ModelP M, float* L, int lane, float fc0, float fc1, float* obs, float fc2 = 0.0f, float fc3 = 0.0f) {
  RobotObs ro;
  float q[4] = {L[L_BASE + 3], L[L_BASE + 4], L[L_BASE + 5], L[L_BASE + 6]};
  quat_to_rp_heading(q, ro.rpy, &ro.cy, &ro.sy);
  ro.rpy[2] = 0.0f;
  const float vx = ro.cy * L[L_BASE + 7] + ro.sy * L[L_BASE + 8], vy = ro.cy * L[L_BASE + 8] - ro.sy * L[L_BASE + 7], vz = L[L_BASE + 9];
  float minz = fminf(L[L_FEET + 2], L[L_FEET + 5]);
  if constexpr (T::NFEET > 2) minz = fminf(minz, fminf(L[L_FEET + 8], L[L_FEET + 11]));
  const float height = L[L_BASE + 2] - minz;
  auto clip5 = [](float x) { return x > 5.f ? 5.f : (x < -5.f ? -5.f : x); };
  float nrm = 0, sp = 0;
  bool fin = true;
  if (lane < T::NJ) {
    const int b = lane + 1;
    const float ang = L[L_Q + b], lo = M->jlo[b], wt = M->jhi[b] - lo;
    nrm = 2 * (ang - lo) / wt - 1;
    sp = 0.1f * L[L_QD + b];
    obs[6 + lane] = clip5(nrm);
    obs[6 + T::NJ + lane] = clip5(sp);
    fin = isfinite(nrm) && isfinite(sp);
  }
  const float head[6] = {height, vx, vy, vz, ro.rpy[0], ro.rpy[1]};
  bool hfin = true;
#pragma unroll
  for (int i = 0; i < 6; ++i) hfin = hfin && isfinite(head[i]);
  if (lane == 0) {
#pragma unroll
    for (int i = 0; i < 6; ++i) obs[i] = clip5(head[i]);
    obs[6 + 2 * T::NJ] = fc0;
    obs[6 + 2 * T::NJ + 1] = fc1;
// ... 425 lines not shown
```

### mocca_envs_amd/csrc/mocca_kernels.h

```cpp
#pragma once
#include <hip/hip_runtime.h>

#include "mocca.h"
#include "mocca_device.h"

namespace MOCCA_NS {

#ifndef MOCCA_WAVES_PER_EU
#define MOCCA_WAVES_PER_EU 4
#endif

DI void flush_obs(const float* L, float* dst, int lane, int obs_dim) {
#pragma unroll 1
  for (int k = lane; k < obs_dim; k += 64) dst[k] = L[L_OBS + k];
}
DI void keep_terminal_obs(const StepArgs& a, const float* L, int env, int lane) {
  wsync();
  if (a.final_obs) flush_obs(L, a.final_obs + (size_t)env * a.obs_dim, lane, a.obs_dim);
  wsync();
}

template <class T>
DI void keep_robot_state(const StepArgs& a, const float* L, int env, int lane) {
  static_assert(ROBOT_OBS<T> <= 64 && ROBOT_OBS<T> <= ROBOT_STATE_STRIDE, "one store per lane");
// ... 142 lines not shown
    if (!(-25.0f < pitch * R2D && pitch * R2D < 25.0f)) posture += fabsf(pitch);
    progress *= 2.0f;
    posture *= 0.2f;
    tall = 2.0f;
    t.done = (t.t > 240 && t.nsi <= 4);
    if (fl.body_touch) { tall = -1.0f; t.done = 1; }
  }
  const int last = MOCCA_MAX_TERRAIN_STEPS - 1;
  float step_bonus = 0.0f, bonus = 0.0f;
  if (reached && t.trc == 1 && t.nsi != last) step_bonus = 50.0f * powf(2.718f, -powf(fdmin, M->step_bonus_smoothness) / 0.25f);
  if ((t.nsi == last || t.stop) && dist < 0.15f) bonus = 2.0f;
  __threadfence_block();
  delta_to_k_targets(M, L, ter, t, ro, lane, obs + ROBOT_OBS<T>);
  if (cur_idx != t.nsi) calc_potential(M, L, t, ro, &dist, &cd, &sd);
  float rew;
  if (!a.random_reward) {
    rew = progress - energy + step_bonus + bonus + tall - posture - joints;
  } else {
    const float terms[8] = {progress, -energy, step_bonus, bonus, 0.0f, tall, -posture, -joints};
    rew = 0.0f;
#pragma unroll
    for (int k = 0; k < 8; ++k) {
      float w;
      if (a.random_reward == 1) {
        w = 0.8f + 0.4f * draw_u<INJECT>(a, env + a.env_offset, t.episode, t.draw + k);
        if (lane == 0) tk[MOCCA_TW_REWARD_WEIGHTS + k] = __float_as_uint(w);
      } else {
        w = __uint_as_float(tk[MOCCA_TW_REWARD_WEIGHTS + k]);
      }
      rew += w * terms[k];
    }
    if (a.random_reward == 1) t.draw += 8;
  }
  t.cover = cover;
  return {rew, t.nsi};
}

template <class T>
DI StepResult cassie_step(const StepArgs& __restrict__ a, ModelP M, float* L, uint32_t* tk, int lane, unsigned long long ppk, TaskRegs& __restrict__ t,
                          float* obs) {
  t.istep += M->n_llc;
  float jv = 0.0f;
  if (lane < M->n_ordered) {
    jv = (L[L_Q + M->ordered_body[lane]] - L[L_Q0 + lane]) / M->control_dt;
    tk[MOCCA_TW_JVEL + lane] = __float_as_uint(jv);
  }
  stage_joints<T, false>(M, L, lane);
  walk_kinematics<T, false>(M, L, lane, ppk);
  wsync();
  t.t += 1;
  const CassieState cs = cassie_state(M, L, lane, t.initz);
  const float old = t.linpot;
  t.linpot = cassie_potential(M, L);
  const float alive = cs.height > M->alive_height ? 2.0f : -1.0f;
  if (!cs.finite || alive < 0.0f) t.done = 1;
  float rew = alive + (t.linpot - old);
  float phase = 0.0f;
  if (M->cassie_mode != MOCCA_CASSIE_PLAIN) {
    const int f1 = traj_frame(a, M, t.istep, &phase);
    rew = cassie_mocap_reward(a, M, L, lane, cs, jv, f1);
  }
  cassie_observe(M, L, lane, cs, t.initz, jv, phase, obs);
  return {rew, 0};
}

template <class T, int TASK, bool INJECT = false>
__global__ __launch_bounds__(64, MOCCA_WAVES_PER_EU) void mocca_step_kernel(StepArgs a) {
  __shared__ float L[L_TOTAL];
  const int lane = threadIdx.x;
  if ((int)blockIdx.x >= a.n_envs) return;
  const int env = a.order ? uni(a.order[blockIdx.x]) : (int)blockIdx.x;
  ModelP M = (ModelP)a.model;
  float* st = a.dyn + (size_t)env * DYN_STRIDE;
  uint32_t* tk = a.task + (size_t)env * MOCCA_TASK_WORDS;
  float* ter = TASK == MOCCA_TASK_WALKER3D_STEPPER ? a.terrain + (size_t)env * TERRAIN_STRIDE : nullptr;
  float* obs_out = a.obs + (size_t)env * a.obs_dim;
  float* obs = L + L_OBS;
  int32_t* dbg = a.dbg ? a.dbg + (size_t)env * MOCCA_DEBUG_WORDS : nullptr;

  const bool warm_ld = INJECT || uni(__float_as_int(M->warmstart)) != 0, warm_st = warm_ld || a.persist_warm != 0;
  if (dbg && lane == 0) { dbg[16] = 0; dbg[17] = 0; dbg[18] = 0; }
  load_dyn(st, L, lane, T::NJ, T::NSLOT, warm_ld);
  pace_start(a, L, lane, INJECT ? 0 : a.pace);
  if (lane == 0) L[L_KEEPWARM] = __int_as_float((warm_st ? 1 : 0) | ((a.prio & PRIO_DELASSUS_VALU) ? 2 : 0));
  const unsigned long long ppk = OUTWARD_ROUNDS<T> ? T::lane_packed(lane) : T::path_packed(lane < T::NB ? lane : 0);
  ContactFlags fl = {0, 0, 0, 0, 0, 0, 0, 0, 0};
  int cover = 0;
  constexpr bool LATE = LATE_ARGS<T, TASK, INJECT>;
  StepArgs late, late_reset;
  const StepArgs& al = LATE ? late : a;
  if constexpr (TASK == MOCCA_TASK_CASSIE) {
    const int no = M->n_ordered, nctl = M->n_ctrl, mode = M->cassie_mode;
    float target = 0.0f;
    if (lane < nctl) {
      float base = M->ctrl_base[lane];
      if (mode != MOCCA_CASSIE_PLAIN) {
        const int f0 = traj_frame(a, M, (int)tk[MOCCA_TW_ISTEP]);
        base = (lane < nctl - 2 && M->residual_control) ? a.traj[(size_t)f0 * MOCCA_TRAJ_STRIDE + M->ctrl_oidx[lane]] : 0.0f;
      }
      target = base + (lane < nctl - 2 ? a.act[(size_t)env * (nctl - 2) + lane] : 0.0f);
    }
    if (lane < no) {
      L[L_JVEL + lane] = __uint_as_float(tk[MOCCA_TW_JVEL + lane]);
      L[L_Q0 + lane] = L[L_Q + M->ordered_body[lane]];
    }
    if (lane < MOCCA_MAX_BODIES) L[L_TAU + lane] = 0.0f;
    if (lane == 0) { L[L_Q] = 0.0f; L[L_QD] = 0.0f; }
    wsync();
    const int nllc = INJECT ? 0 : M->n_llc;
    int last_rows = uni((int)tk[MOCCA_TW_LAST_ROWS]);
    if (!INJECT && a.pace == 0) set_issue_priority(last_rows, a.prio);
#pragma unroll 1
    for (int it = 0; it < nllc; ++it) {
      ModelP Ms = M;
      int ln = lane;
      unsigned long long pk = ppk;
      asm volatile("" : "+s"(Ms), "+v"(ln), "+v"(pk));
      if (ln < no) {
        const float al = Ms->jvel_alpha;
        L[L_JVEL + ln] = (1.0f - al) * L[L_JVEL + ln] + al * L[L_QD + Ms->ordered_body[ln]];
      }
      wsync();
      if (ln < nctl) {
        const int b = Ms->ctrl_body[ln];
        const float perr = target - L[L_Q + b];
        float verr = -L[L_JVEL + Ms->ctrl_oidx[ln]];
        verr = verr < -5.0f ? -5.0f : (verr > 5.0f ? 5.0f : verr);
        const float tq = Ms->ctrl_kp[ln] * perr + Ms->ctrl_kd[ln] * verr, lim = Ms->torque_limit[b];
        L[L_TAU + b] = tq < -lim ? -lim : (tq > lim ? lim : tq);
      }
      wsync();
      substep<T, TASK>(Ms, L, ln, nullptr, 0, pk, dbg, a.prio, last_rows, HeightFieldArgs{nullptr, 0, 0, 0.0f}, it, nllc);
    }
    late_args<LATE>(late);
    if (!INJECT && lane == 0) tk[MOCCA_TW_LAST_ROWS] = (uint32_t)last_rows;
  } else {
    {
      const float applied_gain = __uint_as_float(tk[MOCCA_TW_APPLIED_GAIN]);
      if (lane < T::NJ) {
        const float act_raw = a.act[(size_t)env * T::NJ + lane];
        const float c = act_raw < -1.0f ? -1.0f : (act_raw > 1.0f ? 1.0f : act_raw);
        L[L_TAU + 1 + lane] = M->gain[lane + 1] * applied_gain * c;
      }
    }
    if (lane == 0) { L[L_TAU] = 0.0f; L[L_Q] = 0.0f; L[L_QD] = 0.0f; }
    wsync();

    STAMP(28);
    if constexpr (TASK == MOCCA_TASK_WALKER3D_STEPPER) stage_planks(M, L, lane, ter);
    const int nsub = INJECT ? 0 : M->n_substeps;
    const int nsi0 = TASK == MOCCA_TASK_WALKER3D_STEPPER ? (int)tk[MOCCA_TW_NEXT_STEP_INDEX] : 0;
    int last_rows = uni((int)tk[MOCCA_TW_LAST_ROWS]);
    if (!INJECT && a.pace == 0) set_issue_priority(last_rows, a.prio);
    const float* hfp = a.hf;
    if constexpr (TASK == MOCCA_TASK_WALKER3D_PLANNER) hfp = env_heightfield(a, env);
#pragma unroll 1
    for (int s = 0; s < nsub; ++s) {
      ModelP Ms = M;
      int ln = lane;
      unsigned long long pk = ppk;
      asm volatile("" : "+s"(Ms), "+v"(ln), "+v"(pk));
      fl = substep<T, TASK>(Ms, L, ln, ter, nsi0, pk, dbg, a.prio, last_rows, HeightFieldArgs{hfp, a.hf_rows, a.hf_cols, a.hf_scale}, s, nsub, &cover);
    }
    late_args<LATE>(late);
    if constexpr (INJECT) {
      const int32_t* tc = al.inj_touch + (size_t)env * T::NFEET;
      fl.touch0 = tc[0] != 0; fl.touch1 = tc[1] != 0;
// ... 153 lines not shown
```

### mocca_envs_amd/csrc/topo_cassie.h

```cpp
#pragma once
__device__ static const signed char kPathCassie[19][7] = {
  {-1, -1, -1, -1, -1, -1, -1},
  {1, -1, -1, -1, -1, -1, -1},
  {1, 2, -1, -1, -1, -1, -1},
  {1, 2, 3, -1, -1, -1, -1},
  {1, 2, 3, 4, -1, -1, -1},
  {1, 2, 3, 4, 5, -1, -1},
  {1, 2, 3, 4, 5, 6, -1},
  {1, 2, 3, 4, 5, 6, 7},
  {1, 2, 3, 8, -1, -1, -1},
  {1, 2, 3, 8, 9, -1, -1},
  {10, -1, -1, -1, -1, -1, -1},
  {10, 11, -1, -1, -1, -1, -1},
  {10, 11, 12, -1, -1, -1, -1},
  {10, 11, 12, 13, -1, -1, -1},
  {10, 11, 12, 13, 14, -1, -1},
  {10, 11, 12, 13, 14, 15, -1},
  {10, 11, 12, 13, 14, 15, 16},
  {10, 11, 12, 17, -1, -1, -1},
  {10, 11, 12, 17, 18, -1, -1},
};
__device__ static const signed char kChildCassie[19][2] = {
  {10, 1},
  {2, -1},
  {3, -1},
  {8, 4},
  {5, -1},
  {6, -1},
  {7, -1},
  {-1, -1},
  {9, -1},
  {-1, -1},
  {11, -1},
  {12, -1},
  {17, 13},
  {14, -1},
  {15, -1},
  {16, -1},
  {-1, -1},
  {18, -1},
  {-1, -1},
};
__device__ static const signed char kLevelCassie[8][4] = {
  {-1, -1, -1, -1},
  {1, 10, -1, -1},
  {2, 11, -1, -1},
  {3, 12, -1, -1},
  {4, 13, 8, 17},
  {5, 14, 9, 18},
  {6, 15, -1, -1},
  {7, 16, -1, -1},
};
__device__ static const unsigned long long kPathPkCassie[19] = {0x0ull, 0x1ull, 0x41ull, 0xc41ull, 0x20c41ull, 0x520c41ull, 0xc520c41ull, 0x1cc520c41ull, 0x40c41ull, 0x940c41ull, 0xaull, 0x16aull, 0x316aull, 0x6b16aull, 0xe6b16aull, 0x1ee6b16aull, 0x41ee6b16aull, 0x8b16aull, 0x128b16aull};
__device__ static const unsigned long long kLanePkCassie[64] = {0x400000000000000ull, 0x800000000000001ull, 0xc00000000000041ull, 0x1000000000000c41ull, 0x1400000000020c41ull, 0x1800000000520c41ull, 0x1c0000000c520c41ull, 0x1cc520c41ull, 0x40c41ull, 0x940c41ull, 0xaull, 0x16aull, 0x316aull, 0x6b16aull, 0xe6b16aull, 0x1ee6b16aull, 0x840000041ee6b16aull, 0x880000000008b16aull, 0x8c0000000128b16aull, 0x2000000000000000ull, 0x2400000000000000ull, 0x0ull, 0x0ull, 0x0ull, 0x0ull, 0x0ull, 0x0ull, 0x0ull, 0x0ull, 0x0ull, 0x0ull, 0x0ull, 0x2800000000000000ull, 0x2c00000000000000ull, 0x3000000000000000ull, 0x3400000000000000ull, 0x3800000000000000ull, 0x3c00000000000000ull, 0x4000000000000000ull, 0x0ull, 0x0ull, 0x0ull, 0x0ull, 0x0ull, 0x0ull, 0x0ull, 0x0ull, 0x0ull, 0xa800000000000000ull, 0xac00000000000000ull, 0xb000000000000000ull, 0x4400000000000000ull, 0x4800000000000000ull, 0x0ull, 0x0ull, 0x0ull, 0x0ull, 0x0ull, 0x0ull, 0x0ull, 0x0ull, 0x0ull, 0x0ull, 0x0ull};
struct TopoCassie {
  static constexpr int NB = 19;
  static constexpr int NJ = 18;
  static constexpr int ND = 24;
  static constexpr int MAXD = 7;
  static constexpr int MAXCH = 2;
  static constexpr int MAXW = 4;
  static constexpr int NG = 24;
  static constexpr int NSLOT = 24;
  static constexpr int NPAIR = 0;
  static constexpr int NCLOS = 2;
  static constexpr int NFEET = 2;
  static constexpr int parent(int b) { constexpr int t[19] = {-1, 0, 1, 2, 3, 4, 5, 6, 3, 8, 0, 10, 11, 12, 13, 14, 15, 12, 17}; return t[b]; }
  static constexpr int depth(int b) { constexpr int t[19] = {0, 1, 2, 3, 4, 5, 6, 7, 4, 5, 1, 2, 3, 4, 5, 6, 7, 4, 5}; return t[b]; }
  static constexpr unsigned anc_mask(int b) { constexpr unsigned t[19] = {0x0u, 0x2u, 0x6u, 0xeu, 0x1eu, 0x3eu, 0x7eu, 0xfeu, 0x10eu, 0x30eu, 0x400u, 0xc00u, 0x1c00u, 0x3c00u, 0x7c00u, 0xfc00u, 0x1fc00u, 0x21c00u, 0x61c00u}; return t[b]; }
  static __device__ __forceinline__ int path(int b, int k) { return kPathCassie[b][k]; }
  static __device__ __forceinline__ int child(int b, int k) { return kChildCassie[b][k]; }
  static __device__ __forceinline__ int level(int d, int s) { return kLevelCassie[d][s]; }
  static constexpr int clevel(int d, int s) { constexpr int t[8][4] = {{-1, -1, -1, -1}, {1, 10, -1, -1}, {2, 11, -1, -1}, {3, 12, -1, -1}, {4, 13, 8, 17}, {5, 14, 9, 18}, {6, 15, -1, -1}, {7, 16, -1, -1}}; return t[d][s]; }
  static constexpr bool massless(int b) { constexpr bool t[19] = {false, false, false, false, false, false, false, false, true, false, false, false, false, false, false, false, false, true, false}; return b >= 0 && t[b]; }
  static constexpr int ccarry(int b) { constexpr int t[19] = {-1, 2, 3, 4, 5, 6, 7, -1, 9, -1, 11, 12, 13, 14, 15, 16, -1, 18, -1}; return b < 0 ? -1 : t[b]; }
  static constexpr int cchild(int b, int k) { constexpr int t[19][2] = {{10, 1}, {2, -1}, {3, -1}, {8, 4}, {5, -1}, {6, -1}, {7, -1}, {-1, -1}, {9, -1}, {-1, -1}, {11, -1}, {12, -1}, {17, 13}, {14, -1}, {15, -1}, {16, -1}, {-1, -1}, {18, -1}, {-1, -1}}; return b < 0 ? -1 : t[b][k]; }
  static __device__ __forceinline__ unsigned long long path_packed(int b) { return kPathPkCassie[b]; }
  static constexpr bool OUTWARD_DPP = false;
  static constexpr int out_body(int lane) { constexpr int t[64] = {1, 2, 3, 4, 5, 6, 7, -1, -1, -1, -1, -1, -1, -1, -1, -1, 1, 2, 3, 8, 9, -1, -1, -1, -1, -1, -1, -1, -1, -1, -1, -1, 10, 11, 12, 13, 14, 15, 16, -1, -1, -1, -1, -1, -1, -1, -1, -1, 10, 11, 12, 17, 18, -1, -1, -1, -1, -1, -1, -1, -1, -1, -1, -1}; return t[lane]; }
  static constexpr bool out_primary(int lane) { constexpr bool t[64] = {true, true, true, true, true, true, true, false, false, false, false, false, false, false, false, false, false, false, false, true, true, false, false, false, false, false, false, false, false, false, false, false, true, true, true, true, true, true, true, false, false, false, false, false, false, false, false, false, false, false, false, true, true, false, false, false, false, false, false, false, false, false, false, false}; return t[lane]; }
  static __device__ __forceinline__ unsigned long long lane_packed(int lane) { return kLanePkCassie[lane]; }
  static __device__ __forceinline__ int out_lane(unsigned long long lane_pk) { return (int)(lane_pk >> 58); }
};
```

### mocca_envs_amd/csrc/topo_crab2d.h

```cpp
#pragma once
__device__ static const signed char kPathCrab2D[7][3] = {
  {-1, -1, -1},
  {1, -1, -1},
  {1, 2, -1},
  {1, 2, 3},
  {4, -1, -1},
  {4, 5, -1},
  {4, 5, 6},
};
__device__ static const signed char kChildCrab2D[7][2] = {
  {4, 1},
  {2, -1},
  {3, -1},
  {-1, -1},
  {5, -1},
  {6, -1},
  {-1, -1},
};
__device__ static const signed char kLevelCrab2D[4][4] = {
  {-1, -1, -1, -1},
  {1, 4, -1, -1},
  {2, 5, -1, -1},
  {3, 6, -1, -1},
};
__device__ static const unsigned long long kPathPkCrab2D[7] = {0x0ull, 0x1ull, 0x41ull, 0xc41ull, 0x4ull, 0xa4ull, 0x18a4ull};
__device__ static const unsigned long long kLanePkCrab2D[64] = {0x400000000000000ull, 0x800000000000001ull, 0xc00000000000041ull, 0xc41ull, 0x4ull, 0xa4ull, 0x18a4ull, 0x0ull, 0x0ull, 0x0ull, 0x0ull, 0x0ull, 0x0ull, 0x0ull, 0x0ull, 0x0ull, 0x1000000000000000ull, 0x1400000000000000ull, 0x1800000000000000ull, 0x0ull, 0x0ull, 0x0ull, 0x0ull, 0x0ull, 0x0ull, 0x0ull, 0x0ull, 0x0ull, 0x0ull, 0x0ull, 0x0ull, 0x0ull, 0x0ull, 0x0ull, 0x0ull, 0x0ull, 0x0ull, 0x0ull, 0x0ull, 0x0ull, 0x0ull, 0x0ull, 0x0ull, 0x0ull, 0x0ull, 0x0ull, 0x0ull, 0x0ull, 0x0ull, 0x0ull, 0x0ull, 0x0ull, 0x0ull, 0x0ull, 0x0ull, 0x0ull, 0x0ull, 0x0ull, 0x0ull, 0x0ull, 0x0ull, 0x0ull, 0x0ull, 0x0ull};
struct TopoCrab2D {
  static constexpr int NB = 7;
  static constexpr int NJ = 6;
  static constexpr int ND = 12;
  static constexpr int MAXD = 3;
  static constexpr int MAXCH = 2;
  static constexpr int MAXW = 4;
  static constexpr int NG = 7;
  static constexpr int NSLOT = 14;
  static constexpr int NPAIR = 9;
  static constexpr int NCLOS = 0;
  static constexpr int NFEET = 2;
  static constexpr int parent(int b) { constexpr int t[7] = {-1, 0, 1, 2, 0, 4, 5}; return t[b]; }
  static constexpr int depth(int b) { constexpr int t[7] = {0, 1, 2, 3, 1, 2, 3}; return t[b]; }
  static constexpr unsigned anc_mask(int b) { constexpr unsigned t[7] = {0x0u, 0x2u, 0x6u, 0xeu, 0x10u, 0x30u, 0x70u}; return t[b]; }
  static __device__ __forceinline__ int path(int b, int k) { return kPathCrab2D[b][k]; }
  static __device__ __forceinline__ int child(int b, int k) { return kChildCrab2D[b][k]; }
  static __device__ __forceinline__ int level(int d, int s) { return kLevelCrab2D[d][s]; }
  static constexpr int clevel(int d, int s) { constexpr int t[4][4] = {{-1, -1, -1, -1}, {1, 4, -1, -1}, {2, 5, -1, -1}, {3, 6, -1, -1}}; return t[d][s]; }
  static constexpr bool massless(int b) { constexpr bool t[7] = {false, false, false, false, false, false, false}; return b >= 0 && t[b]; }
  static constexpr int ccarry(int b) { constexpr int t[7] = {-1, 2, 3, -1, 5, 6, -1}; return b < 0 ? -1 : t[b]; }
  static constexpr int cchild(int b, int k) { constexpr int t[7][2] = {{4, 1}, {2, -1}, {3, -1}, {-1, -1}, {5, -1}, {6, -1}, {-1, -1}}; return b < 0 ? -1 : t[b][k]; }
  static __device__ __forceinline__ unsigned long long path_packed(int b) { return kPathPkCrab2D[b]; }
  static constexpr bool OUTWARD_DPP = true;
  static constexpr int out_body(int lane) { constexpr int t[64] = {1, 2, 3, -1, -1, -1, -1, -1, -1, -1, -1, -1, -1, -1, -1, -1, 4, 5, 6, -1, -1, -1, -1, -1, -1, -1, -1, -1, -1, -1, -1, -1, -1, -1, -1, -1, -1, -1, -1, -1, -1, -1, -1, -1, -1, -1, -1, -1, -1, -1, -1, -1, -1, -1, -1, -1, -1, -1, -1, -1, -1, -1, -1, -1}; return t[lane]; }
  static constexpr bool out_primary(int lane) { constexpr bool t[64] = {true, true, true, false, false, false, false, false, false, false, false, false, false, false, false, false, true, true, true, false, false, false, false, false, false, false, false, false, false, false, false, false, false, false, false, false, false, false, false, false, false, false, false, false, false, false, false, false, false, false, false, false, false, false, false, false, false, false, false, false, false, false, false, false}; return t[lane]; }
  static __device__ __forceinline__ unsigned long long lane_packed(int lane) { return kLanePkCrab2D[lane]; }
  static __device__ __forceinline__ int out_lane(unsigned long long lane_pk) { return (int)(lane_pk >> 58); }
};
```

### mocca_envs_amd/csrc/topo_laikago.h

```cpp
#pragma once
__device__ static const signed char kPathLaikago[13][3] = {
  {-1, -1, -1},
  {1, -1, -1},
  {1, 2, -1},
  {1, 2, 3},
  {4, -1, -1},
  {4, 5, -1},
  {4, 5, 6},
  {7, -1, -1},
  {7, 8, -1},
  {7, 8, 9},
  {10, -1, -1},
  {10, 11, -1},
  {10, 11, 12},
};
__device__ static const signed char kChildLaikago[13][4] = {
  {10, 7, 4, 1},
  {2, -1, -1, -1},
  {3, -1, -1, -1},
  {-1, -1, -1, -1},
  {5, -1, -1, -1},
  {6, -1, -1, -1},
  {-1, -1, -1, -1},
  {8, -1, -1, -1},
  {9, -1, -1, -1},
  {-1, -1, -1, -1},
  {11, -1, -1, -1},
  {12, -1, -1, -1},
  {-1, -1, -1, -1},
};
__device__ static const signed char kLevelLaikago[4][4] = {
  {-1, -1, -1, -1},
  {1, 4, 7, 10},
  {2, 5, 8, 11},
  {3, 6, 9, 12},
};
__device__ static const unsigned long long kPathPkLaikago[13] = {0x0ull, 0x1ull, 0x41ull, 0xc41ull, 0x4ull, 0xa4ull, 0x18a4ull, 0x7ull, 0x107ull, 0x2507ull, 0xaull, 0x16aull, 0x316aull};
__device__ static const unsigned long long kLanePkLaikago[64] = {0x400000000000000ull, 0x800000000000001ull, 0xc00000000000041ull, 0xc41ull, 0x4ull, 0xa4ull, 0x18a4ull, 0x7ull, 0x107ull, 0x2507ull, 0xaull, 0x16aull, 0x316aull, 0x0ull, 0x0ull, 0x0ull, 0x1000000000000000ull, 0x1400000000000000ull, 0x1800000000000000ull, 0x0ull, 0x0ull, 0x0ull, 0x0ull, 0x0ull, 0x0ull, 0x0ull, 0x0ull, 0x0ull, 0x0ull, 0x0ull, 0x0ull, 0x0ull, 0x1c00000000000000ull, 0x2000000000000000ull, 0x2400000000000000ull, 0x0ull, 0x0ull, 0x0ull, 0x0ull, 0x0ull, 0x0ull, 0x0ull, 0x0ull, 0x0ull, 0x0ull, 0x0ull, 0x0ull, 0x0ull, 0x2800000000000000ull, 0x2c00000000000000ull, 0x3000000000000000ull, 0x0ull, 0x0ull, 0x0ull, 0x0ull, 0x0ull, 0x0ull, 0x0ull, 0x0ull, 0x0ull, 0x0ull, 0x0ull, 0x0ull, 0x0ull};
struct TopoLaikago {
  static constexpr int NB = 13;
  static constexpr int NJ = 12;
  static constexpr int ND = 18;
  static constexpr int MAXD = 3;
  static constexpr int MAXCH = 4;
  static constexpr int MAXW = 4;
  static constexpr int NG = 32;
  static constexpr int NSLOT = 32;
  static constexpr int NPAIR = 0;
  static constexpr int NCLOS = 0;
  static constexpr int NFEET = 4;
  static constexpr int parent(int b) { constexpr int t[13] = {-1, 0, 1, 2, 0, 4, 5, 0, 7, 8, 0, 10, 11}; return t[b]; }
  static constexpr int depth(int b) { constexpr int t[13] = {0, 1, 2, 3, 1, 2, 3, 1, 2, 3, 1, 2, 3}; return t[b]; }
  static constexpr unsigned anc_mask(int b) { constexpr unsigned t[13] = {0x0u, 0x2u, 0x6u, 0xeu, 0x10u, 0x30u, 0x70u, 0x80u, 0x180u, 0x380u, 0x400u, 0xc00u, 0x1c00u}; return t[b]; }
  static __device__ __forceinline__ int path(int b, int k) { return kPathLaikago[b][k]; }
  static __device__ __forceinline__ int child(int b, int k) { return kChildLaikago[b][k]; }
  static __device__ __forceinline__ int level(int d, int s) { return kLevelLaikago[d][s]; }
  static constexpr int clevel(int d, int s) { constexpr int t[4][4] = {{-1, -1, -1, -1}, {1, 4, 7, 10}, {2, 5, 8, 11}, {3, 6, 9, 12}}; return t[d][s]; }
  static constexpr bool massless(int b) { constexpr bool t[13] = {false, false, false, false, false, false, false, false, false, false, false, false, false}; return b >= 0 && t[b]; }
  static constexpr int ccarry(int b) { constexpr int t[13] = {-1, 2, 3, -1, 5, 6, -1, 8, 9, -1, 11, 12, -1}; return b < 0 ? -1 : t[b]; }
  static constexpr int cchild(int b, int k) { constexpr int t[13][4] = {{10, 7, 4, 1}, {2, -1, -1, -1}, {3, -1, -1, -1}, {-1, -1, -1, -1}, {5, -1, -1, -1}, {6, -1, -1, -1}, {-1, -1, -1, -1}, {8, -1, -1, -1}, {9, -1, -1, -1}, {-1, -1, -1, -1}, {11, -1, -1, -1}, {12, -1, -1, -1}, {-1, -1, -1, -1}}; return b < 0 ? -1 : t[b][k]; }
  static __device__ __forceinline__ unsigned long long path_packed(int b) { return kPathPkLaikago[b]; }
  static constexpr bool OUTWARD_DPP = true;
  static constexpr int out_body(int lane) { constexpr int t[64] = {1, 2, 3, -1, -1, -1, -1, -1, -1, -1, -1, -1, -1, -1, -1, -1, 4, 5, 6, -1, -1, -1, -1, -1, -1, -1, -1, -1, -1, -1, -1, -1, 7, 8, 9, -1, -1, -1, -1, -1, -1, -1, -1, -1, -1, -1, -1, -1, 10, 11, 12, -1, -1, -1, -1, -1, -1, -1, -1, -1, -1, -1, -1, -1}; return t[lane]; }
  static constexpr bool out_primary(int lane) { constexpr bool t[64] = {true, true, true, false, false, false, false, false, false, false, false, false, false, false, false, false, true, true, true, false, false, false, false, false, false, false, false, false, false, false, false, false, true, true, true, false, false, false, false, false, false, false, false, false, false, false, false, false, true, true, true, false, false, false, false, false, false, false, false, false, false, false, false, false}; return t[lane]; }
  static __device__ __forceinline__ unsigned long long lane_packed(int lane) { return kLanePkLaikago[lane]; }
  static __device__ __forceinline__ int out_lane(unsigned long long lane_pk) { return (int)(lane_pk >> 58); }
};
```

### mocca_envs_amd/csrc/topo_walker2d.h

```cpp
#pragma once
__device__ static const signed char kPathWalker2D[8][3] = {
  {-1, -1, -1},
  {1, -1, -1},
  {2, -1, -1},
  {2, 3, -1},
  {2, 3, 4},
  {5, -1, -1},
  {5, 6, -1},
  {5, 6, 7},
};
__device__ static const signed char kChildWalker2D[8][3] = {
  {5, 2, 1},
  {-1, -1, -1},
  {3, -1, -1},
  {4, -1, -1},
  {-1, -1, -1},
  {6, -1, -1},
  {7, -1, -1},
  {-1, -1, -1},
};
__device__ static const signed char kLevelWalker2D[4][4] = {
  {-1, -1, -1, -1},
  {2, 5, 1, -1},
  {3, 6, -1, -1},
  {4, 7, -1, -1},
};
__device__ static const unsigned long long kPathPkWalker2D[8] = {0x0ull, 0x1ull, 0x2ull, 0x62ull, 0x1062ull, 0x5ull, 0xc5ull, 0x1cc5ull};
__device__ static const unsigned long long kLanePkWalker2D[64] = {0x400000000000000ull, 0x1ull, 0x2ull, 0x62ull, 0x1062ull, 0x5ull, 0xc5ull, 0x1cc5ull, 0x0ull, 0x0ull, 0x0ull, 0x0ull, 0x0ull, 0x0ull, 0x0ull, 0x0ull, 0x800000000000000ull, 0xc00000000000000ull, 0x1000000000000000ull, 0x0ull, 0x0ull, 0x0ull, 0x0ull, 0x0ull, 0x0ull, 0x0ull, 0x0ull, 0x0ull, 0x0ull, 0x0ull, 0x0ull, 0x0ull, 0x1400000000000000ull, 0x1800000000000000ull, 0x1c00000000000000ull, 0x0ull, 0x0ull, 0x0ull, 0x0ull, 0x0ull, 0x0ull, 0x0ull, 0x0ull, 0x0ull, 0x0ull, 0x0ull, 0x0ull, 0x0ull, 0x0ull, 0x0ull, 0x0ull, 0x0ull, 0x0ull, 0x0ull, 0x0ull, 0x0ull, 0x0ull, 0x0ull, 0x0ull, 0x0ull, 0x0ull, 0x0ull, 0x0ull, 0x0ull};
struct TopoWalker2D {
  static constexpr int NB = 8;
  static constexpr int NJ = 7;
  static constexpr int ND = 13;
  static constexpr int MAXD = 3;
  static constexpr int MAXCH = 3;
  static constexpr int MAXW = 4;
  static constexpr int NG = 8;
  static constexpr int NSLOT = 15;
  static constexpr int NPAIR = 0;
  static constexpr int NCLOS = 0;
  static constexpr int NFEET = 2;
  static constexpr int parent(int b) { constexpr int t[8] = {-1, 0, 0, 2, 3, 0, 5, 6}; return t[b]; }
  static constexpr int depth(int b) { constexpr int t[8] = {0, 1, 1, 2, 3, 1, 2, 3}; return t[b]; }
  static constexpr unsigned anc_mask(int b) { constexpr unsigned t[8] = {0x0u, 0x2u, 0x4u, 0xcu, 0x1cu, 0x20u, 0x60u, 0xe0u}; return t[b]; }
  static __device__ __forceinline__ int path(int b, int k) { return kPathWalker2D[b][k]; }
  static __device__ __forceinline__ int child(int b, int k) { return kChildWalker2D[b][k]; }
  static __device__ __forceinline__ int level(int d, int s) { return kLevelWalker2D[d][s]; }
  static constexpr int clevel(int d, int s) { constexpr int t[4][4] = {{-1, -1, -1, -1}, {2, 5, 1, -1}, {3, 6, -1, -1}, {4, 7, -1, -1}}; return t[d][s]; }
  static constexpr bool massless(int b) { constexpr bool t[8] = {false, false, false, false, false, false, false, false}; return b >= 0 && t[b]; }
  static constexpr int ccarry(int b) { constexpr int t[8] = {-1, -1, 3, 4, -1, 6, 7, -1}; return b < 0 ? -1 : t[b]; }
  static constexpr int cchild(int b, int k) { constexpr int t[8][3] = {{5, 2, 1}, {-1, -1, -1}, {3, -1, -1}, {4, -1, -1}, {-1, -1, -1}, {6, -1, -1}, {7, -1, -1}, {-1, -1, -1}}; return b < 0 ? -1 : t[b][k]; }
  static __device__ __forceinline__ unsigned long long path_packed(int b) { return kPathPkWalker2D[b]; }
  static constexpr bool OUTWARD_DPP = true;
  static constexpr int out_body(int lane) { constexpr int t[64] = {1, -1, -1, -1, -1, -1, -1, -1, -1, -1, -1, -1, -1, -1, -1, -1, 2, 3, 4, -1, -1, -1, -1, -1, -1, -1, -1, -1, -1, -1, -1, -1, 5, 6, 7, -1, -1, -1, -1, -1, -1, -1, -1, -1, -1, -1, -1, -1, -1, -1, -1, -1, -1, -1, -1, -1, -1, -1, -1, -1, -1, -1, -1, -1}; return t[lane]; }
  static constexpr bool out_primary(int lane) { constexpr bool t[64] = {true, false, false, false, false, false, false, false, false, false, false, false, false, false, false, false, true, true, true, false, false, false, false, false, false, false, false, false, false, false, false, false, true, true, true, false, false, false, false, false, false, false, false, false, false, false, false, false, false, false, false, false, false, false, false, false, false, false, false, false, false, false, false, false}; return t[lane]; }
  static __device__ __forceinline__ unsigned long long lane_packed(int lane) { return kLanePkWalker2D[lane]; }
  static __device__ __forceinline__ int out_lane(unsigned long long lane_pk) { return (int)(lane_pk >> 58); }
};
```

### mocca_envs_amd/csrc/topo_walker3d.h

```cpp
#pragma once
__device__ static const signed char kPathWalker3D[22][8] = {
  {-1, -1, -1, -1, -1, -1, -1, -1},
  {1, -1, -1, -1, -1, -1, -1, -1},
  {1, 2, -1, -1, -1, -1, -1, -1},
  {1, 2, 3, -1, -1, -1, -1, -1},
  {1, 2, 3, 4, -1, -1, -1, -1},
  {1, 2, 3, 4, 5, -1, -1, -1},
  {1, 2, 3, 4, 5, 6, -1, -1},
  {1, 2, 3, 4, 5, 6, 7, -1},
  {1, 2, 3, 4, 5, 6, 7, 8},
  {1, 2, 3, 9, -1, -1, -1, -1},
  {1, 2, 3, 9, 10, -1, -1, -1},
  {1, 2, 3, 9, 10, 11, -1, -1},
  {1, 2, 3, 9, 10, 11, 12, -1},
  {1, 2, 3, 9, 10, 11, 12, 13},
  {14, -1, -1, -1, -1, -1, -1, -1},
  {14, 15, -1, -1, -1, -1, -1, -1},
  {14, 15, 16, -1, -1, -1, -1, -1},
  {14, 15, 16, 17, -1, -1, -1, -1},
  {18, -1, -1, -1, -1, -1, -1, -1},
  {18, 19, -1, -1, -1, -1, -1, -1},
  {18, 19, 20, -1, -1, -1, -1, -1},
  {18, 19, 20, 21, -1, -1, -1, -1},
};
__device__ static const signed char kChildWalker3D[22][3] = {
  {18, 14, 1},
  {2, -1, -1},
  {3, -1, -1},
  {9, 4, -1},
  {5, -1, -1},
  {6, -1, -1},
  {7, -1, -1},
  {8, -1, -1},
  {-1, -1, -1},
  {10, -1, -1},
  {11, -1, -1},
  {12, -1, -1},
  {13, -1, -1},
  {-1, -1, -1},
  {15, -1, -1},
  {16, -1, -1},
  {17, -1, -1},
  {-1, -1, -1},
  {19, -1, -1},
  {20, -1, -1},
  {21, -1, -1},
  {-1, -1, -1},
};
__device__ static const signed char kLevelWalker3D[9][4] = {
  {-1, -1, -1, -1},
  {1, -1, 14, 18},
  {2, -1, 15, 19},
  {3, -1, 16, 20},
  {4, 9, 17, 21},
  {5, 10, -1, -1},
  {6, 11, -1, -1},
  {7, 12, -1, -1},
  {8, 13, -1, -1},
};
__device__ static const unsigned long long kPathPkWalker3D[22] = {0x0ull, 0x1ull, 0x41ull, 0xc41ull, 0x20c41ull, 0x520c41ull, 0xc520c41ull, 0x1cc520c41ull, 0x41cc520c41ull, 0x48c41ull, 0xa48c41ull, 0x16a48c41ull, 0x316a48c41ull, 0x6b16a48c41ull, 0xeull, 0x1eeull, 0x41eeull, 0x8c1eeull, 0x12ull, 0x272ull, 0x5272ull, 0xad272ull};
__device__ static const unsigned long long kLanePkWalker3D[64] = {0x400000000000000ull, 0x800000000000001ull, 0xc00000000000041ull, 0x1000000000000c41ull, 0x1400000000020c41ull, 0x1800000000520c41ull, 0x1c0000000c520c41ull, 0x20000001cc520c41ull, 0x41cc520c41ull, 0x48c41ull, 0xa48c41ull, 0x16a48c41ull, 0x316a48c41ull, 0x6b16a48c41ull, 0xeull, 0x1eeull, 0x84000000000041eeull, 0x880000000008c1eeull, 0x8c00000000000012ull, 0x2400000000000272ull, 0x2800000000005272ull, 0x2c000000000ad272ull, 0x3000000000000000ull, 0x3400000000000000ull, 0x0ull, 0x0ull, 0x0ull, 0x0ull, 0x0ull, 0x0ull, 0x0ull, 0x0ull, 0x3800000000000000ull, 0x3c00000000000000ull, 0x4000000000000000ull, 0x4400000000000000ull, 0x0ull, 0x0ull, 0x0ull, 0x0ull, 0x0ull, 0x0ull, 0x0ull, 0x0ull, 0x0ull, 0x0ull, 0x0ull, 0x0ull, 0x4800000000000000ull, 0x4c00000000000000ull, 0x5000000000000000ull, 0x5400000000000000ull, 0x0ull, 0x0ull, 0x0ull, 0x0ull, 0x0ull, 0x0ull, 0x0ull, 0x0ull, 0x0ull, 0x0ull, 0x0ull, 0x0ull};
struct TopoWalker3D {
  static constexpr int NB = 22;
  static constexpr int NJ = 21;
  static constexpr int ND = 27;
  static constexpr int MAXD = 8;
  static constexpr int MAXCH = 3;
  static constexpr int MAXW = 4;
  static constexpr int NG = 22;
  static constexpr int NSLOT = 34;
  static constexpr int NPAIR = 141;
  static constexpr int NCLOS = 0;
  static constexpr int NFEET = 2;
  static constexpr int parent(int b) { constexpr int t[22] = {-1, 0, 1, 2, 3, 4, 5, 6, 7, 3, 9, 10, 11, 12, 0, 14, 15, 16, 0, 18, 19, 20}; return t[b]; }
  static constexpr int depth(int b) { constexpr int t[22] = {0, 1, 2, 3, 4, 5, 6, 7, 8, 4, 5, 6, 7, 8, 1, 2, 3, 4, 1, 2, 3, 4}; return t[b]; }
  static constexpr unsigned anc_mask(int b) { constexpr unsigned t[22] = {0x0u, 0x2u, 0x6u, 0xeu, 0x1eu, 0x3eu, 0x7eu, 0xfeu, 0x1feu, 0x20eu, 0x60eu, 0xe0eu, 0x1e0eu, 0x3e0eu, 0x4000u, 0xc000u, 0x1c000u, 0x3c000u, 0x40000u, 0xc0000u, 0x1c0000u, 0x3c0000u}; return t[b]; }
  static __device__ __forceinline__ int path(int b, int k) { return kPathWalker3D[b][k]; }
  static __device__ __forceinline__ int child(int b, int k) { return kChildWalker3D[b][k]; }
  static __device__ __forceinline__ int level(int d, int s) { return kLevelWalker3D[d][s]; }
  static constexpr int clevel(int d, int s) { constexpr int t[9][4] = {{-1, -1, -1, -1}, {1, -1, 14, 18}, {2, -1, 15, 19}, {3, -1, 16, 20}, {4, 9, 17, 21}, {5, 10, -1, -1}, {6, 11, -1, -1}, {7, 12, -1, -1}, {8, 13, -1, -1}}; return t[d][s]; }
  static constexpr bool massless(int b) { constexpr bool t[22] = {false, true, false, false, true, true, false, false, false, true, true, false, false, false, true, true, false, false, true, true, false, false}; return b >= 0 && t[b]; }
  static constexpr int ccarry(int b) { constexpr int t[22] = {-1, 2, 3, 4, 5, 6, 7, 8, -1, 10, 11, 12, 13, -1, 15, 16, 17, -1, 19, 20, 21, -1}; return b < 0 ? -1 : t[b]; }
  static constexpr int cchild(int b, int k) { constexpr int t[22][3] = {{18, 14, 1}, {2, -1, -1}, {3, -1, -1}, {9, 4, -1}, {5, -1, -1}, {6, -1, -1}, {7, -1, -1}, {8, -1, -1}, {-1, -1, -1}, {10, -1, -1}, {11, -1, -1}, {12, -1, -1}, {13, -1, -1}, {-1, -1, -1}, {15, -1, -1}, {16, -1, -1}, {17, -1, -1}, {-1, -1, -1}, {19, -1, -1}, {20, -1, -1}, {21, -1, -1}, {-1, -1, -1}}; return b < 0 ? -1 : t[b][k]; }
  static __device__ __forceinline__ unsigned long long path_packed(int b) { return kPathPkWalker3D[b]; }
  static constexpr bool OUTWARD_DPP = true;
  static constexpr int out_body(int lane) { constexpr int t[64] = {1, 2, 3, 4, 5, 6, 7, 8, -1, -1, -1, -1, -1, -1, -1, -1, 1, 2, 3, 9, 10, 11, 12, 13, -1, -1, -1, -1, -1, -1, -1, -1, 14, 15, 16, 17, -1, -1, -1, -1, -1, -1, -1, -1, -1, -1, -1, -1, 18, 19, 20, 21, -1, -1, -1, -1, -1, -1, -1, -1, -1, -1, -1, -1}; return t[lane]; }
  static constexpr bool out_primary(int lane) { constexpr bool t[64] = {true, true, true, true, true, true, true, true, false, false, false, false, false, false, false, false, false, false, false, true, true, true, true, true, false, false, false, false, false, false, false, false, true, true, true, true, false, false, false, false, false, false, false, false, false, false, false, false, true, true, true, true, false, false, false, false, false, false, false, false, false, false, false, false}; return t[lane]; }
  static __device__ __forceinline__ unsigned long long lane_packed(int lane) { return kLanePkWalker3D[lane]; }
  static __device__ __forceinline__ int out_lane(unsigned long long lane_pk) { return (int)(lane_pk >> 58); }
};
```

### mocca_envs_amd/lib.py

```python
from __future__ import annotations

import ctypes as C
import os

HERE = os.path.dirname(os.path.abspath(__file__))
LIB_PATH = os.environ.get("MOCCA_LIB_PATH") or os.path.join(HERE, "libmocca_hip.so")

ABI_VERSION = 8
PARAM_AUTO_RESET, PARAM_EVAL_MODE, PARAM_CURRICULUM, PARAM_RANDOM_POSE, PARAM_HOST_RETARGET, PARAM_SEED, PARAM_ENV_OFFSET, PARAM_APPLIED_GAIN, PARAM_RANDOM_REWARD = 0, 1, 2, 3, 4, 5, 6, 7, 8
PARAM_ISSUE_PRIORITY = 9
PARAM_PERSIST_IMPULSES = 10
PARAM_KERNEL_VARIANT = 11
PARAM_ORDER_EVERY = 12
PARAM_PACE_TICKS = 13
DEBUG_WORDS = 20
CAMERA_FLOATS = 16
RENDER_MAX_SIZE = 4096
SCAN_MAX_POINTS = 256
DEPTH_MAX_PIXELS, DEPTH_STABILISED, DEPTH_SEE_ROBOT = 256, 1, 2
HF_MAX_FIELDS, HF_MAX_PEAKS = 1024, 256
RAND_WORDS, RAND_MAX_DELAY, RAND_MAX_INTERVAL = 4, 7, 65536
RENDER_ID_NONE, RENDER_ID_GROUND, RENDER_ID_PLANK0, RENDER_ID_HEIGHTFIELD, RENDER_ID_TARGET, RENDER_ID_LINK0 = -1, 32, 33, 37, 38, 64

_vp, _i, _u64, _sz, _d = C.c_void_p, C.c_int, C.c_uint64, C.c_size_t, C.c_double
SYMBOLS = {
    "mocca_abi_version": (_i, []),
    "mocca_model_sizeof": (_sz, []),
    "mocca_create": (_i, [_vp, _sz, _i, _i, _i, C.POINTER(_vp)]),
    "mocca_destroy": (_i, [_vp]),
    "mocca_n_envs": (_i, [_vp]),
    "mocca_obs_dim": (_i, [_vp]),
    "mocca_act_dim": (_i, [_vp]),
    "mocca_plan_dim": (_i, [_vp]),
    "mocca_state_dim": (_i, [_vp]),
    "mocca_reset": (_i, [_vp, _vp, _u64, _vp, _vp]),
    "mocca_step": (_i, [_vp, _vp, _vp, _vp, _vp, _vp, _vp]),
    "mocca_task_step": (_i, [_vp] * 10),
    "mocca_set_base_controller": (_i, [_vp, _vp, _sz, _vp, _i, _d]),
    "mocca_set_base_controller_norm": (_i, [_vp, _vp, _vp, _d]),
    "mocca_plan_step": (_i, [_vp, _vp, _vp, _vp, _vp, _vp, _vp]),
    "mocca_get_base_outputs": (_i, [_vp, _vp, _vp, _vp]),
    "mocca_set_draw_tape": (_i, [_vp, _vp, _i]),
    "mocca_observe": (_i, [_vp, _vp, _vp]),
    "mocca_get_state": (_i, [_vp, _vp, _vp]),
    "mocca_set_state": (_i, [_vp, _vp, _vp]),
    "mocca_get_task": (_i, [_vp, _vp, _vp]),
    "mocca_set_task": (_i, [_vp, _vp, _vp]),
    "mocca_get_terrain": (_i, [_vp, _vp, _vp]),
    "mocca_set_terrain": (_i, [_vp, _vp, _vp]),
    "mocca_set_param": (_i, [_vp, _i, _d]),
    "mocca_set_param_v": (_i, [_vp, _i, _vp, _i, _vp]),
    "mocca_set_seed": (_i, [_vp, _u64]),
    "mocca_set_debug_buffer": (_i, [_vp, _vp]),
    "mocca_set_terminal_obs_buffer": (_i, [_vp, _vp]),
    "mocca_set_episode_stats": (_i, [_vp, _vp, _vp, _vp, _vp, _i, _sz]),
    "mocca_episode_serial": (C.c_uint32, [_vp]),
    "mocca_set_trajectory": (_i, [_vp, _vp, _i, _d, _d]),
    "mocca_set_heightfield": (_i, [_vp, _vp, _i, _i, _d]),
    "mocca_set_heightfield_bank": (_i, [_vp, _vp, _i, _i, _i, _d]),
    "mocca_generate_heightfields": (_i, [_vp, _i, _i, _u64, _i, _d, _vp]),
    "mocca_set_env_fields": (_i, [_vp, _vp, _i, _vp]),
    "mocca_get_env_fields": (_i, [_vp, _vp, _vp]),
    "mocca_get_heightfields": (_i, [_vp, _i, _i, _vp, _vp]),
    "mocca_get_link_frames": (_i, [_vp, _vp, _vp]),
    "mocca_render": (_i, [_vp, _vp, _i, _vp, _i, _i, _vp, _vp, _vp, _vp]),
    "mocca_set_height_scan": (_i, [_vp, _vp, _i, _d, _d]),
    "mocca_scan_dim": (_i, [_vp]),
    "mocca_height_scan": (_i, [_vp, _vp, _i, _vp, _vp]),
    "mocca_set_depth_camera": (_i, [_vp, _i, _vp, _i, _i, _d, _d, _d, _i]),
    "mocca_depth_dim": (_i, [_vp]),
    "mocca_depth_camera": (_i, [_vp, _vp, _i, _vp, _vp, _vp]),
    "mocca_set_policy": (_i, [_vp, _vp, _i, _i, _i, _d]),
    "mocca_update_policy": (_i, [_vp, _vp, _sz, _vp]),
    "mocca_act": (_i, [_vp, _vp, _i, _vp, _i, _vp, _vp, _vp, _vp, _vp]),
    "mocca_act_step": (_i, [_vp, _vp, _i, _vp, _i] + [_vp] * 9),
    "mocca_act_plan_step": (_i, [_vp, _vp, _i, _vp, _i] + [_vp] * 9),
    "mocca_set_policy_symmetry": (_i, [_vp, _vp, _vp, _vp, _vp]),
    "mocca_set_policy_mirror_loss": (_i, [_vp, _vp, _vp, _vp, _vp, _d]),
    "mocca_set_policy_mirror_dup": (_i, [_vp, _vp, _vp, _vp, _vp]),
    "mocca_gae": (_i, [_vp, _vp, _vp, _vp, _vp, _i, _d, _d, _d, _vp, _vp, _i, _d, _vp, _vp]),
    "mocca_obs_stats": (_i, [_vp, _vp, C.c_int64, _i, _i, _vp, _d, _vp, _vp, _vp]),
    "mocca_ppo_grad": (_i, [_vp, _vp, _i, _vp, _vp, _vp, _vp, _vp, _vp, C.c_int64, _d, _d, _d, _i, _vp, _vp, _vp]),
    "mocca_ppo_grad_sym": (_i, [_vp, _vp, _i, _vp, _vp, _vp, _vp, _vp, _vp, C.c_int64, _d, _d, _d, _i, _vp, _vp, _vp]),
    "mocca_ppo_grad_mirror": (_i, [_vp, _vp, _i, _vp, _vp, _vp, _vp, _vp, _vp, C.c_int64, _d, _d, _d, _i, _vp, _vp, _vp]),
    "mocca_ppo_grad_dup": (_i, [_vp, _vp, _i, _vp, _vp, _vp, _vp, _vp, _vp, C.c_int64, _d, _d, _d, _i, _vp, _vp, _vp]),
    "mocca_adam_step": (_i, [_vp, _vp, _sz, _vp, C.c_int64, _vp, _vp, _d, _d, _d, _d, _d, _vp]),
    "mocca_ppo_update": (_i, [_vp, _vp, _i, _vp, _vp, _vp, _vp, _vp, C.c_int64, C.c_int64, _i, _d, _d, _d, _i, _vp, _sz, C.c_int64, _vp, _vp,
                              _d, _d, _d, _d, _d, _u64, _vp, _vp]),
    "mocca_distill_grad": (_i, [_vp, _vp, _i, _vp, _vp, _vp, C.c_int64, _d, _d, _vp, _vp, _vp]),
    "mocca_distill_update": (_i, [_vp, _vp, _i, _vp, _vp, C.c_int64, C.c_int64, _i, _d, _d, _vp, _sz, C.c_int64, _vp, _vp,
                                  _d, _d, _d, _d, _d, _u64, _vp, _vp]),
    "mocca_set_teacher": (_i, [_vp, _vp, _i, _i, _i, _d]),
    "mocca_update_teacher": (_i, [_vp, _vp, _sz, _vp]),
    "mocca_teacher_act": (_i, [_vp, _vp, _i, C.c_int64, _vp, _vp, _vp]),
    "mocca_set_policy_priv": (_i, [_vp, _vp, _i, _i, _i, _i, _d]),
    "mocca_set_critic_rows": (_i, [_vp, _vp, _i]),
# ... 57 lines not shown
```

### mocca_envs_amd/model.py

```python
from __future__ import annotations

import ctypes as C
import math
from dataclasses import dataclass, field
from types import SimpleNamespace
from typing import Dict, List, Optional, Sequence, Tuple

import numpy as np

MAX_BODIES = 24
MAX_GEOMS = 32
MAX_PAIRS = 192
MAX_FEET = 4
MAX_SLOTS = 40
MAGIC = 0x41434F4D
VERSION = 13

GEOM_SPHERE, GEOM_CAPSULE = 0, 1
TASK_WALKER3D_CUSTOM, TASK_WALKER3D_STEPPER, TASK_CASSIE, TASK_WALKER3D_PLANNER = 0, 1, 2, 3
TASK_WORDS = 40
TASK_RECORD = (
    ("WALK_TARGET_X", 0, 1, "f"), ("WALK_TARGET_Y", 1, 1, "f"), ("WALK_TARGET_Z", 2, 1, "f"),
    ("LINEAR_POTENTIAL", 3, 1, "f"), ("ANGULAR_POTENTIAL", 4, 1, "f"), ("CLOSE_COUNT", 5, 1, "i"), ("STOP_FRAMES", 6, 1, "f"),
    ("DONE", 7, 1, "i"), ("T", 8, 1, "i"), ("EPISODE", 9, 1, "i"), ("DRAW", 10, 1, "i"), ("MIRRORED", 11, 1, "i"),
# ... 920 lines not shown
        _put(m.init_vel, (0.8, 0.0, 0.0))
    return m.finalize_tables()


LAIKAGO_JOINTS = ["%s_%s" % (leg, j) for leg in ("FR", "FL", "RR", "RL")
                  for j in ("hip_motor_2_chassis_joint", "upper_leg_2_hip_motor_joint", "lower_leg_2_upper_leg_joint")]
LAIKAGO_FEET = ["toeFR", "toeFL", "toeRR", "toeRL"]
LAIKAGO_SHAPE_MARGIN = 0.001


def compile_laikago(stepper: bool = False, plank_class: str = "LargePlank") -> MoccaModel:
    from . import laikago_table as LT

    def contents(link, R, t):
        e = LT.LINKS[link]
        parts, geoms = [], []
        if e["mass"] > 0.0:
            if e["sphere"] is not None:
                I = np.eye(3) * 0.4 * e["mass"] * e["sphere"]["radius"] ** 2
            else:
                Ri = R @ _rpy_mat(e["rpy"])
                hx, hy, hz = (h + LAIKAGO_SHAPE_MARGIN for h in e["box_half"])
                I = Ri @ np.diag([hy * hy + hz * hz, hx * hx + hz * hz, hx * hx + hy * hy]) @ Ri.T * (e["mass"] / 3.0)
            parts.append((e["mass"], R @ np.asarray(e["com"], float) + t, I))
        fr = e["friction"] if e["friction"] is not None else 1.0
        if e["sphere"] is not None:
            g = _urdf_point(R @ np.asarray(e["sphere"]["center"], float) + t, e["sphere"]["radius"], fr)
            if link in LAIKAGO_FEET:
                g.foot, g.margin_key, g.margin_weight = LAIKAGO_FEET.index(link), link, (1.0, g.p1)
            geoms.append(g)
        geoms += [_urdf_point(R @ np.asarray(p, float) + t, 0.0, fr) for p in e["points"]]
        return parts, geoms

    ch = LT.LINKS["chassis"]
    R0 = _rpy_mat(ch["rpy"]).T
    links = _urdf_links(LT, "chassis", contents, R0, -R0 @ np.asarray(ch["com"], float))
    assert [link.name for link in links[1:]] == LAIKAGO_JOINTS
    feet = {g.foot: (b, g.p1) for b, link in enumerate(links) for g in link.geoms if g.foot >= 0}
    m = _assemble(links, [feet[k] for k in range(len(LAIKAGO_FEET))])
    for b in range(1, m.n_bodies):
        m.gain[b] = 40.0
        m.init_q[b] = -math.pi / 6 if links[b].name.endswith("lower_leg_2_upper_leg_joint") else 0.0
    m.dt, m.n_substeps = (1.0 / 240.0, 4) if stepper else (1.0 / 480.0, 8)
    _put(m.init_pos, (0.25, 0.0, 0.53) if stepper else (0.0, 0.0, 0.56))
    m.init_quat[3] = 1.0
    _set_walker_task(m, termination_height=0.0)
    _set_mirror(m, [0, 1, 2, 6, 7, 8], [3, 4, 5, 9, 10, 11])
    m.task_flags |= TASKF_BODY_CONTACT
    if stepper:
        _put(m.init_vel, (0.5, 0.0, 0.25))
        set_stepper_params(m, quadruped=True, plank_class=plank_class)
        m.task_flags = (m.task_flags & ~TASKF_BODY_CONTACT) | TASKF_QUADRUPED_STEPPER
    return m.finalize_tables()


def joint_limits(m: MoccaModel) -> Tuple[np.ndarray, np.ndarray]:
    nj = m.n_joints
    lo = np.array([m.jlo[b] for b in range(1, nj + 1)], dtype=np.float32)
    hi = np.array([m.jhi[b] for b in range(1, nj + 1)], dtype=np.float32)
    return lo, hi


OUTWARD_ROWS, OUTWARD_ROW_LANES = 4, 16
OUTWARD_SHIFT = 58


def outward_layout(parent: List[int], n_closures: int = 0) -> Tuple[bool, List[int]]:
    nb = len(parent)
    lanes = [-1] * (OUTWARD_ROWS * OUTWARD_ROW_LANES)
    chains = []
    for leaf in (b for b in range(1, nb) if b not in parent[1:]):
        c, cur = [], leaf
        while cur > 0:
            c.append(cur)
            cur = parent[cur]
        chains.append(c[::-1])
    if len(chains) > OUTWARD_ROWS or any(len(c) > OUTWARD_ROW_LANES for c in chains):
        return False, lanes
    for r, c in enumerate(chains):
        lanes[OUTWARD_ROW_LANES * r:OUTWARD_ROW_LANES * r + len(c)] = c
    return n_closures == 0, lanes


def topology_header(m: MoccaModel, name: str = "Walker3D") -> str:
    nb = m.n_bodies
    parent = [m.parent[b] for b in range(nb)]
    depth = [m.depth[b] for b in range(nb)]
    maxd = max(depth)
    children = [[c for c in range(nb) if parent[c] == b] for b in range(nb)]
    maxc = max(len(c) for c in children)
    by_depth = [[b for b in range(nb) if depth[b] == d] for d in range(maxd + 1)]
    maxw = max(4, max(len(l) for l in by_depth[1:]))
    slot_of, carry = {}, [-1] * nb
    levels = [[-1] * maxw for _ in range(maxd + 1)]
    for d in range(maxd, 0, -1):
        taken = set()
        for b in by_depth[d]:
            for c in sorted(children[b]):
                if slot_of[c] not in taken:
                    slot_of[b], carry[b] = slot_of[c], c
                    taken.add(slot_of[c])
                    break
        for b in by_depth[d]:
            if b not in slot_of:
                slot_of[b] = min(set(range(maxw)) - taken)
                taken.add(slot_of[b])
        for b in by_depth[d]:
            levels[d][slot_of[b]] = b
    path = []
    for b in range(nb):
        p, cur = [], b
        while cur > 0:
            p.append(cur)
            cur = parent[cur]
        p = p[::-1]
        path.append(p + [-1] * (maxd - len(p)))
    outward_dpp, out_lanes = outward_layout(parent, m.n_closures)
    out_primary = [b >= 0 and out_lanes.index(b) == l for l, b in enumerate(out_lanes)]
    out_lane_bits = [0 if b < 0 else b + (0 if p else 32) for b, p in zip(out_lanes, out_primary)]
    pathpk = [sum(((path[b][k] if path[b][k] >= 0 else 0) << (5 * k)) for k in range(maxd)) for b in range(nb)]
    assert 5 * maxd <= OUTWARD_SHIFT and nb <= 32, "the packed path and the outward pass's lane bits share one 64-bit word"

    def arr(vals):
        return "{" + ", ".join(str(v) for v in vals) + "}"

    lines = [
        "// GENERATED by mocca_envs_amd.model.topology_header() -- do not edit.",
        "// Kinematic tree of %s as compile-time tables (numbers live in the MoccaModel blob)." % name,
        "#pragma once",
        "// runtime-indexed copies (per-lane lookups)",
        "__device__ static const signed char kPath%s[%d][%d] = {" % (name, nb, maxd),
    ]
    lines += ["  %s," % arr(p) for p in path]
    lines += ["};", "__device__ static const signed char kChild%s[%d][%d] = {" % (name, nb, maxc)]
    lines += ["  %s," % arr(sorted(c, reverse=True) + [-1] * (maxc - len(c))) for c in children]
    lines += ["};", "__device__ static const signed char kLevel%s[%d][%d] = {" % (name, maxd + 1, maxw)]
    lines += ["  %s," % arr(l) for l in levels]
    lines += [
        "};",
        "__device__ static const unsigned long long kPathPk%s[%d] = %s;" % (
            name, nb, arr(["0x%xull" % v for v in pathpk])),
        "// per LANE: the packed path of the lane's body in the lane = body layout (kPathPk of body `lane`, 0 behind the last body) and, in the top six",
        "// bits, the lane's body in the level-by-level ABA outward pass (model.py outward_layout): + 32 on a lane that repeats a shared trunk, 0 idle",
        "__device__ static const unsigned long long kLanePk%s[%d] = %s;" % (
            name, len(out_lanes), arr(["0x%xull" % ((pathpk[l] if l < nb else 0) | (ol << OUTWARD_SHIFT)) for l, ol in enumerate(out_lane_bits)])),
        "struct Topo%s {" % name,
        "  static constexpr int NB = %d;        // bodies incl. floating base" % nb,
        "  static constexpr int NJ = %d;        // hinges" % (nb - 1),
        "  static constexpr int ND = %d;        // generalised velocities" % (nb + 5),
        "  static constexpr int MAXD = %d;      // tree depth" % maxd,
        "  static constexpr int MAXCH = %d;     // children per body" % maxc,
        "  static constexpr int MAXW = %d;      // bodies per level" % maxw,
        "  static constexpr int NG = %d;        // geoms" % m.n_geoms,
        "  static constexpr int NSLOT = %d;     // terrain contact slots" % m.n_slots,
        "  static constexpr int NPAIR = %d;     // self-collision candidate pairs" % m.n_pairs,
        "  static constexpr int NCLOS = %d;     // point-to-point loop closures" % m.n_closures,
        "  static constexpr int NFEET = %d;     // feet (entries of the observation, robots.py:74-86)" % m.n_feet,
        "  // constexpr functions (implicitly __host__ __device__ under hipcc) fold after unrolling",
        "  static constexpr int parent(int b) { constexpr int t[%d] = %s; return t[b]; }" % (nb, arr(parent)),
        "  static constexpr int depth(int b) { constexpr int t[%d] = %s; return t[b]; }" % (nb, arr(depth)),
        "  static constexpr unsigned anc_mask(int b) { constexpr unsigned t[%d] = %s; return t[b]; }"
        % (nb, arr(["0x%xu" % m.anc_mask[b] for b in range(nb)])),
        "  static __device__ __forceinline__ int path(int b, int k) { return kPath%s[b][k]; }" % name,
        "  static __device__ __forceinline__ int child(int b, int k) { return kChild%s[b][k]; }" % name,
        "  static __device__ __forceinline__ int level(int d, int s) { return kLevel%s[d][s]; }" % name,
        "  // compile-time versions: with the loops over k / d unrolled these cost a few VALU ops and NO memory access",
        "  // (a dependent global table load per tree level / path step is what dominated the latency-bound phases)",
        "  static constexpr int clevel(int d, int s) { constexpr int t[%d][%d] = {%s}; return t[d][s]; }"
        % (maxd + 1, maxw, ", ".join(arr(l) for l in levels)),
        "  // links without mass or inertia (the intermediate links of multi-hinge joints): a tree level that holds only such links skips the",
        "  // reads of its (all-zero) link inertia and bias force in the ABA inward pass; mocca_create() checks the blob against this table",
        "  static constexpr bool massless(int b) { constexpr bool t[%d] = %s; return b >= 0 && t[b]; }"
        % (nb, arr(["true" if (m.mass[b] == 0.0 and all(m.inertia[b][i] == 0.0 for i in range(6)) and b > 0) else "false" for b in range(nb)])),
        "  // the child whose articulated inertia stays in registers (same slot, next level), -1 if none",
        "  static constexpr int ccarry(int b) { constexpr int t[%d] = %s; return b < 0 ? -1 : t[b]; }" % (nb, arr(carry)),
        "  static constexpr int cchild(int b, int k) { constexpr int t[%d][%d] = {%s}; return b < 0 ? -1 : t[b][k]; }"
        % (nb, maxc, ", ".join(arr(sorted(c, reverse=True) + [-1] * (maxc - len(c))) for c in children)),
        "  // the lane's own root->body path, 5 bits per step (0 = past the end: joints are numbered from 1): loaded once per kernel, two VGPRs, then",
        "  // every path step is a v_bfe -- no table access inside the walks",
        "  static __device__ __forceinline__ unsigned long long path_packed(int b) { return kPathPk%s[b]; }" % name,
        "  // ABA outward pass, level by level: every root->leaf chain on consecutive lanes from the start of a 16-lane DPP row, so a body's parent is",
        "  // the lane to its left (model.py outward_layout).  out_body: the lane's body, -1 idle; out_primary: the one lane of a body that stores",
        "  // (a trunk that chains share is repeated in their rows); OUTWARD_DPP: at most four chains of at most 16 bodies and no loop closures",
        "  static constexpr bool OUTWARD_DPP = %s;" % ("true" if outward_dpp else "false"),
        "  static constexpr int out_body(int lane) { constexpr int t[%d] = %s; return t[lane]; }" % (len(out_lanes), arr(out_lanes)),
        "  static constexpr bool out_primary(int lane) { constexpr bool t[%d] = %s; return t[lane]; }"
        % (len(out_lanes), arr(["true" if p else "false" for p in out_primary])),
        "  // what the step kernel keeps per lane across the substeps: path_packed of body `lane` (0 behind the last body), out_lane above it",
        "  static __device__ __forceinline__ unsigned long long lane_packed(int lane) { return kLanePk%s[lane]; }" % name,
        "  static __device__ __forceinline__ int out_lane(unsigned long long lane_pk) { return (int)(lane_pk >> %d); }" % OUTWARD_SHIFT,
        "};",
        "",
    ]
    return "\n".join(lines)


def write_topology_headers(outdir: Optional[str] = None) -> None:
    import os
    outdir = outdir or os.path.join(os.path.dirname(os.path.abspath(__file__)), "csrc")
    with open(os.path.join(outdir, "topo_walker3d.h"), "w") as f:
        f.write(topology_header(compile_walker3d(), "Walker3D"))
    with open(os.path.join(outdir, "topo_cassie.h"), "w") as f:
        f.write(topology_header(compile_cassie(), "Cassie"))
    with open(os.path.join(outdir, "topo_walker2d.h"), "w") as f:
        f.write(topology_header(compile_walker2d(), "Walker2D"))
    with open(os.path.join(outdir, "topo_crab2d.h"), "w") as f:
        f.write(topology_header(compile_crab2d(), "Crab2D"))
    with open(os.path.join(outdir, "topo_laikago.h"), "w") as f:
        f.write(topology_header(compile_laikago(), "Laikago"))


if __name__ == "__main__":
    write_topology_headers()
```

Measured before the change: 44.86 million env-steps/s.

## Split constraint-row outward sweep across paired lane groups for Walker3D

Result: no change. 45.21 million env-steps/s, median of 6 (+0.8%).

```diff
diff --git a/include/mocca.h b/include/mocca.h
--- a/include/mocca.h
+++ b/include/mocca.h
@@ -37,6 +37,7 @@
   MOCCA_PARAM_KERNEL_VARIANT = 11,
   MOCCA_PARAM_ORDER_EVERY = 12,
   MOCCA_PARAM_PACE_TICKS = 13,
+  MOCCA_PARAM_SWEEP_ONE_LANE = 14,
 };
 
 #define MOCCA_DEBUG_WORDS 20
diff --git a/mocca_envs_amd/csrc/mocca_api.hip b/mocca_envs_amd/csrc/mocca_api.hip
--- a/mocca_envs_amd/csrc/mocca_api.hip
+++ b/mocca_envs_amd/csrc/mocca_api.hip
@@ -104,6 +104,7 @@
   bool wide = false;
   int force_full = 0;
   bool delassus_valu = false;
+  bool sweep_one_lane = false;
   int persist_warm = 0;
   int pace = -18;
   DevBuf<unsigned long long> d_pace_acc;
@@ -515,7 +516,7 @@
   a.gain_v = h->pvec_on[2] ? h->d_pvec[2].get() : nullptr;
   a.gain = h->gain;
   a.dbg = h->dbg;
-  a.prio = h->prio | (h->delassus_valu ? PRIO_DELASSUS_VALU : 0);
+  a.prio = h->prio | (h->delassus_valu ? PRIO_DELASSUS_VALU : 0) | (h->sweep_one_lane ? PRIO_SWEEP_ONE_LANE : 0);
   a.traj = h->d_traj; a.traj_n = h->traj_n; a.traj_tmax = h->traj_tmax; a.traj_cstep = h->traj_cstep;
   a.final_obs = h->final_obs;
   a.persist_warm = h->persist_warm;
@@ -1152,6 +1153,9 @@
       if (inst == 1 && h->wide) { h->err = "MOCCA_PARAM_KERNEL_VARIANT = 1: this blob needs the 64-row instance (caps beyond 48 rows / 12 contacts, or sweep_alternate)"; return MOCCA_E_ARG; }
       h->force_full = inst; h->delassus_valu = ((int)value & 4) != 0; break;
     }
+    case MOCCA_PARAM_SWEEP_ONE_LANE:
+      if (value != 0.0 && value != 1.0) { h->err = "MOCCA_PARAM_SWEEP_ONE_LANE is 0 or 1"; return MOCCA_E_ARG; }
+      h->sweep_one_lane = value != 0.0; break;
     default: h->err = "unknown parameter id"; return MOCCA_E_ARG;
   }
   return MOCCA_OK;
diff --git a/mocca_envs_amd/csrc/mocca_device.h b/mocca_envs_amd/csrc/mocca_device.h
--- a/mocca_envs_amd/csrc/mocca_device.h
+++ b/mocca_envs_amd/csrc/mocca_device.h
@@ -224,6 +224,12 @@
 #else
 constexpr bool WALK_LEVELS = OUTWARD_ROUNDS<T>;
 #endif
+template <class T, int TASK>
+#ifdef MOCCA_NO_TRIM_10
+constexpr bool SWEEP_SPLIT = false;
+#else
+constexpr bool SWEEP_SPLIT = T::SWEEP_PAIRS && !COMPACT && MAXR == 48 && TASK == MOCCA_TASK_WALKER3D_CUSTOM;
+#endif
 template <class T>
 constexpr int walk_base_lane() {
   for (int l = 63; l >= 0; --l)
@@ -250,6 +256,16 @@
 DI float dot6(const float* a, const float* b) {
   return a[0] * b[0] + a[1] * b[1] + a[2] * b[2] + a[3] * b[3] + a[4] * b[4] + a[5] * b[5];
 }
+DI float sweep_dot6(const float* U, const float* a, int order, unsigned partner = 0u) {
+  float t0 = 0.0f, t1 = 0.0f, t;
+  if (order != 0) { t0 = U[0] * a[0]; t0 = __builtin_fmaf(U[1], a[1], t0); }
+  if (order != 1) { t1 = a[1] * U[1]; t1 = __builtin_fmaf(a[0], U[0], t1); }
+  if (order == 2) t = __uint_as_float((__float_as_uint(t1) & partner) | (__float_as_uint(t0) & ~partner));
+  else t = order == 1 ? t0 : t1;
+#pragma unroll
+  for (int i = 2; i < 6; ++i) t = __builtin_fmaf(a[i], U[i], t);
+  return t;
+}
 DI void matvec3(const float* R, const float* x, float* o) {
   float a = R[0] * x[0] + R[1] * x[1] + R[2] * x[2];
   float b = R[3] * x[0] + R[4] * x[1] + R[5] * x[2];
@@ -309,6 +325,9 @@
 DI float rsq(float x) { return __builtin_amdgcn_rsqf(x); }
 DI void pin6(float* v) { asm volatile("" : "+v"(v[0]), "+v"(v[1]), "+v"(v[2]), "+v"(v[3]), "+v"(v[4]), "+v"(v[5])); }
 DI void pin1(float& v) { asm volatile("" : "+v"(v)); }
+DI float row_down(float v) {
+  return __builtin_bit_cast(float, __builtin_amdgcn_ds_swizzle(__builtin_bit_cast(int, v), 0x000F));
+}
 template <int CTRL>
 DI float dpp_mov(float v) {
   return __builtin_bit_cast(float, __builtin_amdgcn_update_dpp(0, __builtin_bit_cast(int, v), CTRL, 0xF, 0xF, true));
@@ -1475,6 +1494,7 @@
 #define MOCCA_DELASSUS_MFMA_MIN 8
 #endif
 constexpr int PRIO_DELASSUS_VALU = 1 << 18;
+constexpr int PRIO_SWEEP_ONE_LANE = 1 << 19;
 enum : int { L_DX = L_V };
 static_assert(L_DX + 28 * DELASSUS_MFMA_ROWS <= L_J && MAXR >= DELASSUS_MFMA_ROWS, "the X rows of the matrix-pipe Delassus build end before the J rows");
 template <int R, int C>
@@ -1706,7 +1726,7 @@
     dbg[16] = (int32_t)(unsigned)h; dbg[17] = (int32_t)(unsigned)(h >> 32); dbg[18] += 1;
   }
 }
-template <class T, bool MATRIX_PIPE>
+template <class T, bool MATRIX_PIPE, bool SPLIT>
 DI void solve_constraints(ModelP M, float* L, int lane, int nc_found, int nc_wanted, unsigned long long ppk, int32_t* dbg, const float* Afac, int prio, int& rows_out) {
   const int wave_flags = uni(__float_as_int(L[L_KEEPWARM]));
   const bool keep_warm = (wave_flags & 1) != 0;
@@ -1934,7 +1954,70 @@
 #pragma unroll
     for (int i = 0; i < 6; ++i) X[i] = a0[i];
   }
-  {
+  bool split = false;
+  if constexpr (SPLIT) split = r_fr <= 16 && nc <= 8 && !(wave_flags & 4);
+  if (split) {
+    if constexpr (SPLIT) {
+      constexpr int NS = T::SWEEP_STEPS;
+      static_assert(MAXR == 48 && !COMPACT, "the friction rows of 8 contacts sit on lanes 32 .. 47");
+      const unsigned pm = (unsigned)__builtin_amdgcn_sbfe(lane, 4, 1);
+      float ab[6], qu[T::MAXD], qub[T::MAXD];
+#pragma unroll
+      for (int i = 0; i < 6; ++i) { ab[i] = row_down(a0[i]); X[i] = ab[i]; }
+#pragma unroll
+      for (int k = 0; k < T::MAXD; ++k) qu[k] = row_down(pu[k]);
+      const unsigned qa = __float_as_uint(row_down(__uint_as_float(ma)));
+      unsigned qb = 0u;
+      if (two_paths) {
+#pragma unroll
+        for (int k = 0; k < T::MAXD; ++k) qub[k] = row_down(pub[k]);
+        qb = __float_as_uint(row_down(__uint_as_float(mb)));
+      }
+      float acs[NS][6], qs[NS];
+      int dl = 0;
+      const float* Lp = L2;
+      unsigned mas = qa, mbs = qb;
+#pragma unroll
+      for (int s = 0; s < NS; ++s) {
+        const int b = T::sweep_body(0, s), ps = T::sweep_pstep(s);
+        if (T::sweep_body(1, s) - b != dl) {
+          dl = T::sweep_body(1, s) - b;
+          Lp = L2 + (int)(pm & (unsigned)(SVS * dl));
+          mas = qa >> (pm & (unsigned)dl);
+          if (two_paths) mbs = qb >> (pm & (unsigned)dl);
+        }
+        const bool inner = has_child<T>(b);
+        const float* ap = ps < 0 ? ab : acs[ps < 0 ? 0 : ps];
+        float U[6];
+#pragma unroll
+        for (int i = 0; i < 6; ++i) U[i] = Lp[L_SV + SVS * b + SV_V + i];
+        const int dpos = T::depth(b) - 1;
+        float ub = __uint_as_float(__float_as_uint(qu[dpos]) & (unsigned)__builtin_amdgcn_sbfe((int)mas, b, 1));
+        if (two_paths) ub += __uint_as_float(__float_as_uint(qub[dpos]) & (unsigned)__builtin_amdgcn_sbfe((int)mbs, b, 1));
+        const float qdd = ub - sweep_dot6(U, ap, b != 1 ? 0 : (T::sweep_body(1, s) == 1 ? 1 : 2), pm);
+        qs[s] = qdd;
+        if (inner) {
+          float S[6];
+#pragma unroll
+          for (int i = 0; i < 6; ++i) { S[i] = Lp[L_SV + SVS * b + i]; acs[s][i] = __builtin_fmaf(S[i], qdd, ap[i]); }
+          pin6(acs[s]);
+        }
+        pin1(qs[s]);
+      }
+#pragma unroll
+      for (int s = 0; s < NS; ++s) {
+        if (T::sweep_owned(s)) {
+          unsigned idle;
+          asm volatile("" : "=v"(idle));
+          const auto sw = __builtin_amdgcn_permlane16_swap(__float_as_uint(qs[s]), idle, false, false);
+          X[5 + T::sweep_body(0, s)] = __uint_as_float(sw[0]);
+          X[5 + T::sweep_body(1, s)] = __uint_as_float(sw[1]);
+        } else {
+          X[5 + T::sweep_body(0, s)] = qs[s];
+        }
+      }
+    }
+  } else {
     float acc[T::NB][6];
 #pragma unroll
     for (int i = 0; i < 6; ++i) acc[0][i] = a0[i];
@@ -1952,12 +2035,18 @@
       const int dpos = T::depth(b) - 1;
       float ub = __uint_as_float(__float_as_uint(pu[dpos]) & (unsigned)__builtin_amdgcn_sbfe((int)ma, b, 1));
       if (two_paths) ub += __uint_as_float(__float_as_uint(pub[dpos]) & (unsigned)__builtin_amdgcn_sbfe((int)mb, b, 1));
-      const float qdd = ub - dot6(U, acc[p]);
+      float qdd;
+      if constexpr (SPLIT) qdd = ub - sweep_dot6(U, acc[p], b == 1 ? 1 : 0);
+      else qdd = ub - dot6(U, acc[p]);
       X[5 + b] = qdd;
       if (inner) {
         float S[6];
 #pragma unroll
-        for (int i = 0; i < 6; ++i) { S[i] = L2[L_SV + SVS * b + i]; acc[b][i] = acc[p][i] + S[i] * qdd; }
+        for (int i = 0; i < 6; ++i) {
+          S[i] = L2[L_SV + SVS * b + i];
+          if constexpr (SPLIT) acc[b][i] = __builtin_fmaf(S[i], qdd, acc[p][i]);
+          else acc[b][i] = acc[p][i] + S[i] * qdd;
+        }
         pin6(acc[b]);
       }
       pin1(X[5 + b]);
@@ -2216,7 +2305,7 @@
   STAMP(2);
   pace_checkpoint(L, done0 + 36, total);
 #ifndef MOCCA_SKIP_SOLVE
-  solve_constraints<T, !PLANNER48>(M, L, lane, nc, nc_wanted, ppk, dbg, Afac, prio, rows_out);
+  solve_constraints<T, !PLANNER48, SWEEP_SPLIT<T, TASK>>(M, L, lane, nc, nc_wanted, ppk, dbg, Afac, prio, rows_out);
 #endif
   if (dbg) { __builtin_amdgcn_s_waitcnt(0); dbg_fold_step(dbg, lane); }
   STAMP(3);
diff --git a/mocca_envs_amd/csrc/mocca_kernels.h b/mocca_envs_amd/csrc/mocca_kernels.h
--- a/mocca_envs_amd/csrc/mocca_kernels.h
+++ b/mocca_envs_amd/csrc/mocca_kernels.h
@@ -248,7 +248,7 @@
   if (dbg && lane == 0) { dbg[16] = 0; dbg[17] = 0; dbg[18] = 0; }
   load_dyn(st, L, lane, T::NJ, T::NSLOT, warm_ld);
   pace_start(a, L, lane, INJECT ? 0 : a.pace);
-  if (lane == 0) L[L_KEEPWARM] = __int_as_float((warm_st ? 1 : 0) | ((a.prio & PRIO_DELASSUS_VALU) ? 2 : 0));
+  if (lane == 0) L[L_KEEPWARM] = __int_as_float((warm_st ? 1 : 0) | ((a.prio & PRIO_DELASSUS_VALU) ? 2 : 0) | ((a.prio & PRIO_SWEEP_ONE_LANE) ? 4 : 0));
   const unsigned long long ppk = OUTWARD_ROUNDS<T> ? T::lane_packed(lane) : T::path_packed(lane < T::NB ? lane : 0);
   ContactFlags fl = {0, 0, 0, 0, 0, 0, 0, 0, 0};
   int cover = 0;
diff --git a/mocca_envs_amd/csrc/topo_cassie.h b/mocca_envs_amd/csrc/topo_cassie.h
--- a/mocca_envs_amd/csrc/topo_cassie.h
+++ b/mocca_envs_amd/csrc/topo_cassie.h
@@ -79,6 +79,11 @@
   static constexpr bool OUTWARD_DPP = false;
   static constexpr int out_body(int lane) { constexpr int t[64] = {1, 2, 3, 4, 5, 6, 7, -1, -1, -1, -1, -1, -1, -1, -1, -1, 1, 2, 3, 8, 9, -1, -1, -1, -1, -1, -1, -1, -1, -1, -1, -1, 10, 11, 12, 13, 14, 15, 16, -1, -1, -1, -1, -1, -1, -1, -1, -1, 10, 11, 12, 17, 18, -1, -1, -1, -1, -1, -1, -1, -1, -1, -1, -1}; return t[lane]; }
   static constexpr bool out_primary(int lane) { constexpr bool t[64] = {true, true, true, true, true, true, true, false, false, false, false, false, false, false, false, false, false, false, false, true, true, false, false, false, false, false, false, false, false, false, false, false, true, true, true, true, true, true, true, false, false, false, false, false, false, false, false, false, false, false, false, true, true, false, false, false, false, false, false, false, false, false, false, false}; return t[lane]; }
+  static constexpr bool SWEEP_PAIRS = false;
+  static constexpr int SWEEP_STEPS = 1;
+  static constexpr int sweep_body(int g, int s) { constexpr int t[2][1] = {{0}, {0}}; return t[g][s]; }
+  static constexpr int sweep_pstep(int s) { constexpr int t[1] = {-1}; return t[s]; }
+  static constexpr bool sweep_owned(int s) { constexpr bool t[1] = {false}; return t[s]; }
   static __device__ __forceinline__ unsigned long long lane_packed(int lane) { return kLanePkCassie[lane]; }
   static __device__ __forceinline__ int out_lane(unsigned long long lane_pk) { return (int)(lane_pk >> 58); }
 };
diff --git a/mocca_envs_amd/csrc/topo_crab2d.h b/mocca_envs_amd/csrc/topo_crab2d.h
--- a/mocca_envs_amd/csrc/topo_crab2d.h
+++ b/mocca_envs_amd/csrc/topo_crab2d.h
@@ -51,6 +51,11 @@
   static constexpr bool OUTWARD_DPP = true;
   static constexpr int out_body(int lane) { constexpr int t[64] = {1, 2, 3, -1, -1, -1, -1, -1, -1, -1, -1, -1, -1, -1, -1, -1, 4, 5, 6, -1, -1, -1, -1, -1, -1, -1, -1, -1, -1, -1, -1, -1, -1, -1, -1, -1, -1, -1, -1, -1, -1, -1, -1, -1, -1, -1, -1, -1, -1, -1, -1, -1, -1, -1, -1, -1, -1, -1, -1, -1, -1, -1, -1, -1}; return t[lane]; }
   static constexpr bool out_primary(int lane) { constexpr bool t[64] = {true, true, true, false, false, false, false, false, false, false, false, false, false, false, false, false, true, true, true, false, false, false, false, false, false, false, false, false, false, false, false, false, false, false, false, false, false, false, false, false, false, false, false, false, false, false, false, false, false, false, false, false, false, false, false, false, false, false, false, false, false, false, false, false}; return t[lane]; }
+  static constexpr bool SWEEP_PAIRS = true;
+  static constexpr int SWEEP_STEPS = 3;
+  static constexpr int sweep_body(int g, int s) { constexpr int t[2][3] = {{1, 2, 3}, {4, 5, 6}}; return t[g][s]; }
+  static constexpr int sweep_pstep(int s) { constexpr int t[3] = {-1, 0, 1}; return t[s]; }
+  static constexpr bool sweep_owned(int s) { constexpr bool t[3] = {true, true, true}; return t[s]; }
   static __device__ __forceinline__ unsigned long long lane_packed(int lane) { return kLanePkCrab2D[lane]; }
   static __device__ __forceinline__ int out_lane(unsigned long long lane_pk) { return (int)(lane_pk >> 58); }
 };
diff --git a/mocca_envs_amd/csrc/topo_laikago.h b/mocca_envs_amd/csrc/topo_laikago.h
--- a/mocca_envs_amd/csrc/topo_laikago.h
+++ b/mocca_envs_amd/csrc/topo_laikago.h
@@ -63,6 +63,11 @@
   static constexpr bool OUTWARD_DPP = true;
   static constexpr int out_body(int lane) { constexpr int t[64] = {1, 2, 3, -1, -1, -1, -1, -1, -1, -1, -1, -1, -1, -1, -1, -1, 4, 5, 6, -1, -1, -1, -1, -1, -1, -1, -1, -1, -1, -1, -1, -1, 7, 8, 9, -1, -1, -1, -1, -1, -1, -1, -1, -1, -1, -1, -1, -1, 10, 11, 12, -1, -1, -1, -1, -1, -1, -1, -1, -1, -1, -1, -1, -1}; return t[lane]; }
   static constexpr bool out_primary(int lane) { constexpr bool t[64] = {true, true, true, false, false, false, false, false, false, false, false, false, false, false, false, false, true, true, true, false, false, false, false, false, false, false, false, false, false, false, false, false, true, true, true, false, false, false, false, false, false, false, false, false, false, false, false, false, true, true, true, false, false, false, false, false, false, false, false, false, false, false, false, false}; return t[lane]; }
+  static constexpr bool SWEEP_PAIRS = true;
+  static constexpr int SWEEP_STEPS = 6;
+  static constexpr int sweep_body(int g, int s) { constexpr int t[2][6] = {{1, 2, 3, 7, 8, 9}, {4, 5, 6, 10, 11, 12}}; return t[g][s]; }
+  static constexpr int sweep_pstep(int s) { constexpr int t[6] = {-1, 0, 1, -1, 3, 4}; return t[s]; }
+  static constexpr bool sweep_owned(int s) { constexpr bool t[6] = {true, true, true, true, true, true}; return t[s]; }
   static __device__ __forceinline__ unsigned long long lane_packed(int lane) { return kLanePkLaikago[lane]; }
   static __device__ __forceinline__ int out_lane(unsigned long long lane_pk) { return (int)(lane_pk >> 58); }
 };
diff --git a/mocca_envs_amd/csrc/topo_walker2d.h b/mocca_envs_amd/csrc/topo_walker2d.h
--- a/mocca_envs_amd/csrc/topo_walker2d.h
+++ b/mocca_envs_amd/csrc/topo_walker2d.h
@@ -53,6 +53,11 @@
   static constexpr bool OUTWARD_DPP = true;
   static constexpr int out_body(int lane) { constexpr int t[64] = {1, -1, -1, -1, -1, -1, -1, -1, -1, -1, -1, -1, -1, -1, -1, -1, 2, 3, 4, -1, -1, -1, -1, -1, -1, -1, -1, -1, -1, -1, -1, -1, 5, 6, 7, -1, -1, -1, -1, -1, -1, -1, -1, -1, -1, -1, -1, -1, -1, -1, -1, -1, -1, -1, -1, -1, -1, -1, -1, -1, -1, -1, -1, -1}; return t[lane]; }
   static constexpr bool out_primary(int lane) { constexpr bool t[64] = {true, false, false, false, false, false, false, false, false, false, false, false, false, false, false, false, true, true, true, false, false, false, false, false, false, false, false, false, false, false, false, false, true, true, true, false, false, false, false, false, false, false, false, false, false, false, false, false, false, false, false, false, false, false, false, false, false, false, false, false, false, false, false, false}; return t[lane]; }
+  static constexpr bool SWEEP_PAIRS = true;
+  static constexpr int SWEEP_STEPS = 4;
+  static constexpr int sweep_body(int g, int s) { constexpr int t[2][4] = {{1, 2, 3, 4}, {1, 5, 6, 7}}; return t[g][s]; }
+  static constexpr int sweep_pstep(int s) { constexpr int t[4] = {-1, -1, 1, 2}; return t[s]; }
+  static constexpr bool sweep_owned(int s) { constexpr bool t[4] = {false, true, true, true}; return t[s]; }
   static __device__ __forceinline__ unsigned long long lane_packed(int lane) { return kLanePkWalker2D[lane]; }
   static __device__ __forceinline__ int out_lane(unsigned long long lane_pk) { return (int)(lane_pk >> 58); }
 };
diff --git a/mocca_envs_amd/csrc/topo_walker3d.h b/mocca_envs_amd/csrc/topo_walker3d.h
--- a/mocca_envs_amd/csrc/topo_walker3d.h
+++ b/mocca_envs_amd/csrc/topo_walker3d.h
@@ -86,6 +86,11 @@
   static constexpr bool OUTWARD_DPP = true;
   static constexpr int out_body(int lane) { constexpr int t[64] = {1, 2, 3, 4, 5, 6, 7, 8, -1, -1, -1, -1, -1, -1, -1, -1, 1, 2, 3, 9, 10, 11, 12, 13, -1, -1, -1, -1, -1, -1, -1, -1, 14, 15, 16, 17, -1, -1, -1, -1, -1, -1, -1, -1, -1, -1, -1, -1, 18, 19, 20, 21, -1, -1, -1, -1, -1, -1, -1, -1, -1, -1, -1, -1}; return t[lane]; }
   static constexpr bool out_primary(int lane) { constexpr bool t[64] = {true, true, true, true, true, true, true, true, false, false, false, false, false, false, false, false, false, false, false, true, true, true, true, true, false, false, false, false, false, false, false, false, true, true, true, true, false, false, false, false, false, false, false, false, false, false, false, false, true, true, true, true, false, false, false, false, false, false, false, false, false, false, false, false}; return t[lane]; }
+  static constexpr bool SWEEP_PAIRS = true;
+  static constexpr int SWEEP_STEPS = 12;
+  static constexpr int sweep_body(int g, int s) { constexpr int t[2][12] = {{1, 2, 3, 4, 5, 6, 7, 8, 14, 15, 16, 17}, {1, 2, 3, 9, 10, 11, 12, 13, 18, 19, 20, 21}}; return t[g][s]; }
+  static constexpr int sweep_pstep(int s) { constexpr int t[12] = {-1, 0, 1, 2, 3, 4, 5, 6, -1, 8, 9, 10}; return t[s]; }
+  static constexpr bool sweep_owned(int s) { constexpr bool t[12] = {false, false, false, true, true, true, true, true, true, true, true, true}; return t[s]; }
   static __device__ __forceinline__ unsigned long long lane_packed(int lane) { return kLanePkWalker3D[lane]; }
   static __device__ __forceinline__ int out_lane(unsigned long long lane_pk) { return (int)(lane_pk >> 58); }
 };
diff --git a/mocca_envs_amd/lib.py b/mocca_envs_amd/lib.py
--- a/mocca_envs_amd/lib.py
+++ b/mocca_envs_amd/lib.py
@@ -12,6 +12,7 @@
 PARAM_PERSIST_IMPULSES = 10
 PARAM_KERNEL_VARIANT = 11
 PARAM_ORDER_EVERY = 12
+PARAM_SWEEP_ONE_LANE = 14
 PARAM_PACE_TICKS = 13
 DEBUG_WORDS = 20
 CAMERA_FLOATS = 16
diff --git a/mocca_envs_amd/model.py b/mocca_envs_amd/model.py
--- a/mocca_envs_amd/model.py
+++ b/mocca_envs_amd/model.py
@@ -1026,6 +1026,48 @@
     return n_closures == 0, lanes
 
 
+def sweep_pairs(parent: List[int], n_closures: int = 0) -> Tuple[bool, List[int], List[int], List[int], List[bool]]:
+    refused = (False, [0], [0], [-1], [False])
+    ok, lanes = outward_layout(parent, n_closures)
+    if not ok:
+        return refused
+    chains = [[b for b in lanes[OUTWARD_ROW_LANES * r:OUTWARD_ROW_LANES * (r + 1)] if b >= 0] for r in range(OUTWARD_ROWS)]
+    chains = [c for c in chains if c]
+    pairs, free = [], list(range(len(chains)))
+    while free:
+        i = free.pop(0)
+        j = next((k for k in free if len(chains[k]) == len(chains[i])), None)
+        if j is None:
+            pairs.append((i, i))
+            continue
+        free.remove(j)
+        pairs.append((i, j))
+    if all(i == j for i, j in pairs):
+        return refused
+    P, Q, pstep, owned = [], [], [], []
+    for i, j in pairs:
+        for bp, bq in zip(chains[i], chains[j]):
+            if bp in P and bq in Q:
+                if P.index(bp) != Q.index(bq):
+                    return refused
+                continue
+            if bp in P or bq in Q:
+                return refused
+            pp = -1 if parent[bp] == 0 else (P.index(parent[bp]) if parent[bp] in P else None)
+            pq = -1 if parent[bq] == 0 else (Q.index(parent[bq]) if parent[bq] in Q else None)
+            if pp is None or pp != pq or bq < bp:
+                return refused
+            P.append(bp); Q.append(bq); pstep.append(pp)
+    for s, (bp, bq) in enumerate(zip(P, Q)):
+        if bq in P and bq != bp:
+            return refused
+        owned.append(bq not in P)
+    owners = P + [bq for bq, o in zip(Q, owned) if o]
+    if sorted(owners) != list(range(1, len(parent))):
+        return refused
+    return True, P, Q, pstep, owned
+
+
 def topology_header(m: MoccaModel, name: str = "Walker3D") -> str:
     nb = m.n_bodies
     parent = [m.parent[b] for b in range(nb)]
@@ -1061,6 +1103,7 @@
         path.append(p + [-1] * (maxd - len(p)))
     outward_dpp, out_lanes = outward_layout(parent, m.n_closures)
     out_primary = [b >= 0 and out_lanes.index(b) == l for l, b in enumerate(out_lanes)]
+    sp_ok, sp_p, sp_q, sp_ps, sp_own = sweep_pairs(parent, m.n_closures)
     out_lane_bits = [0 if b < 0 else b + (0 if p else 32) for b, p in zip(out_lanes, out_primary)]
     pathpk = [sum(((path[b][k] if path[b][k] >= 0 else 0) << (5 * k)) for k in range(maxd)) for b in range(nb)]
     assert 5 * maxd <= OUTWARD_SHIFT and nb <= 32, "the packed path and the outward pass's lane bits share one 64-bit word"
@@ -1130,6 +1173,15 @@
         "  static constexpr int out_body(int lane) { constexpr int t[%d] = %s; return t[lane]; }" % (len(out_lanes), arr(out_lanes)),
         "  static constexpr bool out_primary(int lane) { constexpr bool t[%d] = %s; return t[lane]; }"
         % (len(out_lanes), arr(["true" if p else "false" for p in out_primary])),
+        "  // Outward sweep of the constraint rows, a row's lane (group 0) and the lane 16 above it (group 1) in lockstep (model.py sweep_pairs):",
+        "  // sweep_body: the group's body at a step; sweep_pstep: the step that walked the parent, -1 = the base; sweep_owned: group 1's value is",
+        "  // the body's entry of X (false: a trunk both walk, group 0's is).  SWEEP_PAIRS: OUTWARD_DPP and the chains pair off by length",
+        "  static constexpr bool SWEEP_PAIRS = %s;" % ("true" if sp_ok else "false"),
+        "  static constexpr int SWEEP_STEPS = %d;" % len(sp_p),
+        "  static constexpr int sweep_body(int g, int s) { constexpr int t[2][%d] = {%s, %s}; return t[g][s]; }" % (len(sp_p), arr(sp_p), arr(sp_q)),
+        "  static constexpr int sweep_pstep(int s) { constexpr int t[%d] = %s; return t[s]; }" % (len(sp_p), arr(sp_ps)),
+        "  static constexpr bool sweep_owned(int s) { constexpr bool t[%d] = %s; return t[s]; }"
+        % (len(sp_p), arr(["true" if o else "false" for o in sp_own])),
         "  // what the step kernel keeps per lane across the substeps: path_packed of body `lane` (0 behind the last body), out_lane above it",
         "  static __device__ __forceinline__ unsigned long long lane_packed(int lane) { return kLanePk%s[lane]; }" % name,
         "  static __device__ __forceinline__ int out_lane(unsigned long long lane_pk) { return (int)(lane_pk >> %d); }" % OUTWARD_SHIFT,
```
